# steidani/ConTrack

Hardware: AMD Instinct MI355X
Metric: timesteps/sec labeled+tracked (higher is better)
Workload: dtype f32 compare / int32 labels / int64 exact areas

## Files before the change

### contrack_amd/_native.py

```python
import ctypes as C
import os
import weakref

import numpy as np

from . import _abi

_HERE = os.path.dirname(os.path.abspath(__file__))
LIB_PATH = os.environ.get("CTK_LIB", os.path.join(_HERE, "libcontrack_hip.so"))
INCLUDE_DIR = os.environ.get("CTK_INCLUDE", os.path.join(os.path.dirname(_HERE), "include"))
_lib = None

CMP_OPS = {">=": 0, "ge": 0, "<=": 1, "le": 1, ">": 2, "gt": 2, "<": 3, "lt": 3}
GORL_ERRMSG = ' Please select from [>, >=, <, >=] for gorl'

TIMER_NAMES = ["k_threshold", "k_scan", "k_label2d", "k_overlap", "k_extent", "k_run_values", "k_relabel",
               "k_resolve", "k_resolve_final", "k_count", "host_seam_driver", "d2h", "h2d", "total"]


class ContrackHipError(RuntimeError):
    pass


def _headers():
# ... 150 lines not shown

def _subset_table(table):
    off, ids = table
    off, ids = np.ascontiguousarray(off, dtype=np.int64), np.ascontiguousarray(ids, dtype=np.int32)
    if off.ndim != 1 or ids.ndim != 1 or len(off) < 2:
        raise ValueError("a table is (off, ids): off int64 with 2 or T + 1 entries, ids int32")
    return off, ids


def _subset_kind(kind):
    if kind not in SUBSET_KINDS:
        raise ValueError("kind={!r}: 'id' or 'mask'".format(kind))
    return SUBSET_KINDS[kind]


class _SubsetCall:

    def __init__(self, table, invert, kind, want_hits=True):
        self.off, self.ids = _subset_table(table)
        self.hits = np.zeros(len(self.ids), dtype=np.uint64) if want_hits else None
        self.n = C.c_int64(0)
        self.table = (self.off.ctypes.data, len(self.off), self.ids.ctypes.data, len(self.ids), int(bool(invert)), _subset_kind(kind))

    def counts(self):
        return _ptr(self.hits), C.byref(self.n)


BLOCKSTAT_FORMS = ("row_lds", "row_glb")
BLOCK_WANTS = {"shape": ABI.constants["CTK_BLOCK_SHAPE"], "peaks": ABI.constants["CTK_BLOCK_PEAKS"]}
BLOCK_ROW = _dtype("ctk_block_row")


def _block_want(want):
    if isinstance(want, (int, np.integer)):
        return int(want)
    names = (want,) if isinstance(want, str) else tuple(want)
    unknown = [w for w in names if w not in BLOCK_WANTS]
    if unknown or not names:
        raise ValueError("want={!r}: 'shape', 'peaks' or both".format(want))
    return sum(BLOCK_WANTS[w] for w in set(names))


def blockstat_plan(want, longest, ny, nx, steps=1, elem_bytes=4, aligned=True, grid_max=0):
    v = np.zeros(14, dtype=np.int64)
    check(lib().ctk_debug_blockstat_plan(_block_want(want), int(elem_bytes), int(longest), int(ny), int(nx), int(steps), int(bool(aligned)), int(grid_max),
                                         v.ctypes.data))
    return dict(zip(("form", "vec", "vpt", "lds", "bps", "blocks", "grid", "xcd", "passes", "words", "entry", "lds_budget", "lds_entries", "part_lanes"),
                    (int(a) for a in v)))


class _BlockstatCall:

    def __init__(self, table, want):
        self.off, self.ids = _subset_table(table)
        self.rows = np.zeros(len(self.ids), dtype=BLOCK_ROW)
        self.args = (self.off.ctypes.data, len(self.off), self.ids.ctypes.data, len(self.ids), _block_want(want), self.rows.ctypes.data)


def lwa_plan(elem_bytes, rows, nx, ndom=1, steps=1, aligned=True):
    v = np.zeros(12, dtype=np.int64)
    check(lib().ctk_debug_lwa_plan(int(elem_bytes), int(rows), int(nx), int(ndom), int(steps), int(bool(aligned)), v.ctypes.data))
    return dict(zip(("ok", "vec", "strip", "nstrips", "lds", "lds_sel", "blocks", "grid", "xcd", "sel_blocks", "sel_grid", "sel_xcd"), (int(a) for a in v)))


def composite_plan(elem_bytes, npix, unroll=-1):
    v = np.zeros(3, dtype=np.int64)
    check(lib().ctk_debug_composite_plan(int(elem_bytes), int(npix), int(unroll), v.ctypes.data))
    return dict(unroll=int(v[0]), blocks=int(v[1]), grid=int(v[2]))


def centred_plan(elem_bytes, nbins, hy, hx, max_bin=0, kept=None, form=-1, unroll=-1, threads=-1):
    v = np.zeros(6, dtype=np.int64)
    check(lib().ctk_debug_centred_plan(int(elem_bytes), int(nbins), int(hy), int(hx), int(max_bin), int(max_bin if kept is None else kept), int(form),
                                       int(unroll), int(threads), v.ctypes.data))
    return dict(form=int(v[5]), unroll=int(v[0]), threads=int(v[1]), parts=int(v[2]), blocks=int(v[3]), grid=int(v[4]))


def forms(T, ny, nx, nt=None, aligned16=True, async_passes=24, n_cus=256, **query):
    q = FormQuery(T=T, nt=T if nt is None else nt, ny=ny, nx=nx, aligned16=int(aligned16), async_passes=async_passes, n_cus=n_cus,
                  **{k: int(v) for k, v in query.items()})
    p = FormPlan()
    check(lib().ctk_debug_forms(C.byref(q), C.byref(p)))
    return {n: getattr(p, n) for n, _ in FormPlan._fields_}


def debug_live():
    out = (C.c_int64 * 4)()
    check(lib().ctk_debug_live(out))
    return tuple(out)


def lib():
    global _lib
    if _lib is not None:
        return _lib
    if not os.path.exists(LIB_PATH):
        raise ContrackHipError(
            "libcontrack_hip.so not found at %s -- build it with `python -c 'import __graft_entry__ as g; g.build()'` "
            "or `make -C contrack_amd/csrc`; the HIP path has no CPU fallback" % LIB_PATH)
    L = C.CDLL(LIB_PATH)
    missing = [name for name in ABI.functions if not hasattr(L, name)]
    if missing:
        raise ContrackHipError("%s does not export %s, which the headers in %s declare" % (LIB_PATH, ", ".join(missing), INCLUDE_DIR))
    for name, (restype, argtypes) in ABI.functions.items():
        fn = getattr(L, name)
        fn.restype, fn.argtypes = restype, argtypes
    _lib = L
    return L


def _seg_starts(segments):
    st = np.asarray(segments)
    if st.ndim != 1 or (st.size and st.dtype.kind not in "iu"):
        raise ValueError("segment starts must be a 1-D integer array")
    return np.ascontiguousarray(st, dtype=np.int64)


def _thr_or_field(thr, T):
    if thr is None:
        return None
    thr = np.ascontiguousarray(thr, dtype=np.float64)
    if thr.shape != (T,):
        raise ValueError("thr must have shape (T,) and wrow (ny,)")
    return thr


def _groups(group, T, ngroups=None):
    if group is None:
        return None, 1 if ngroups is None else int(ngroups)
    g = np.asarray(group)
    if g.ndim != 1 or g.shape[0] != T:
        raise ValueError("group must hold one id per timestep (%d), not shape %s" % (T, g.shape))
    if g.dtype.kind not in "iu":
        raise ValueError("group ids must be integers")
    if g.size and (g.min() < np.iinfo(np.int32).min or g.max() > np.iinfo(np.int32).max):
        raise ValueError("group ids beyond int32")
    g = np.ascontiguousarray(g, dtype=np.int32)
    return g, (int(g.max()) + 1 if g.size else 1) if ngroups is None else int(ngroups)


def _level_weights(weights, nlev):
    w = np.ascontiguousarray(weights, dtype=np.float64)
    if w.ndim != 1 or w.shape[0] != nlev:
        raise ValueError("weights must hold one value per level (%d), not shape %s" % (nlev, w.shape))
    if not np.all(np.isfinite(w)) or np.any(w < 0):
        raise ValueError("each weight must be finite and >= 0")
    if not np.any(w > 0):
        raise ValueError("all weights are zero: no level is selected")
    return w


def _reversal_rows(rows, ny):
    second = rows.get("eq2") is not None
    if second != (rows.get("tS2") is not None):
        raise ValueError("eq2 and tS2 go together (both or neither)")
    keep = []
    for key, dt in (("eq", np.int32), ("po", np.int32), ("eq2", np.int32), ("dE", np.float64), ("tS", np.float64), ("tN", np.float64), ("tS2", np.float64)):
        if key in ("eq2", "tS2") and not second:
            keep.append(None)
            continue
        a = np.ascontiguousarray(rows[key], dtype=dt)
        if a.shape != (ny,):
            raise ValueError("rows[%r] must hold one value per latitude row (%d), not shape %s" % (key, ny, a.shape))
        keep.append(a)
    return [_ptr(a) for a in keep], keep

# ... 1599 lines not shown
            if not isinstance(field_source, np.memmap) or field_source.dtype not in (np.float32, np.float64):
                field_source = np.ascontiguousarray(field_source, dtype=np.float64 if np.asarray(field_source).dtype == np.float64 else np.float32)
            if field_source.ndim != 3:
                raise ValueError("field must be (time, lat, lon)")
        if shape is None:
            have = [a.shape for a in (flag_source, field_source) if not callable(a)]
            if not have:
                raise ValueError("reader callbacks need shape=(T, ny, nx) and dtype")
            shape = have[0]
        T, ny, nx = (int(v) for v in shape)
        for a in (flag_source, field_source):
            if not callable(a) and a.shape != (T, ny, nx):
                raise ValueError("flag and field must share one (time, lat, lon) shape")
        if callable(field_source):
            if dtype is None:
                raise ValueError("a field reader needs dtype")
            dt = np.dtype(dtype)
        else:
            dt = field_source.dtype
        if dt not in (np.dtype(np.float32), np.dtype(np.float64)):
            raise ValueError("the field must be float32 or float64")
        wrow = np.ascontiguousarray(wrow, dtype=np.float32)
        if wrow.shape != (ny,):
            raise ValueError("wrow must have shape (ny,)")
        tr = _Trampolines()

        def pk(_user, rows, n, idx, nidx):
            view = np.ctypeslib.as_array(C.cast(rows, C.POINTER(C.c_byte)), shape=(n * LIFE_ROW.itemsize,)).view(LIFE_ROW)
            chosen = np.ascontiguousarray(pick(view), dtype=np.int64).reshape(-1)
            if len(chosen) > n:
                raise ValueError("pick returned more indices than rows")
            np.ctypeslib.as_array(C.cast(idx, C.POINTER(C.c_int64)), shape=(max(int(n), 1),))[:len(chosen)] = chosen
            C.cast(nidx, C.POINTER(C.c_int64))[0] = len(chosen)
        pcb = tr.wrap(LIFE_PICK_FN, pk) if pick is not None else LIFE_PICK_FN()
        n, nx_ = C.c_int64(0), C.c_int64(0)
        tail = (wrow.ctypes.data, int(chunk_steps), pcb, None, C.byref(n), C.byref(nx_))
        if arrays:
            fn = L.ctk_lifecycle_stream_f64 if dt == np.float64 else L.ctk_lifecycle_stream_f32
            rc = fn(self._h, flag_source.ctypes.data, field_source.ctypes.data, T, ny, nx, *tail)
        else:
            fcb, vcb = tr.reader(flag_source, C.c_int32, (ny, nx)), tr.reader(field_source, _float_ctype(dt), (ny, nx))
            rc = L.ctk_lifecycle_stream_cb(self._h, dt.itemsize, T, ny, nx, fcb, None, vcb, None, *tail)
        tr.finish(rc)
        rows = self._life_rows(int(n.value))
        idx = np.empty(int(nx_.value), dtype=np.int64)
        exact = np.empty(int(nx_.value), dtype=LIFE_EXACT)
        check(L.ctk_lifecycle_stream_exact(self._h, idx.ctypes.data, exact.ctypes.data, len(idx)))
        return rows, idx, exact

    def debug_lifecycle_path(self, T):
        v = np.zeros(8, dtype=np.int64)
        steps = np.zeros(max(int(T), 1), dtype=np.uint8)
        check(lib().ctk_debug_lifecycle_path(self._h, v.ctypes.data, steps.ctypes.data, int(T)))
        return dict(zip("rw nsx nby vec given_up launches attempts sort".split(), (int(x) for x in v))), steps[:int(T)]

    def lifecycle_dev(self, flag_dev, field_dev, T, ny, nx, wrow, f64=False):
        wrow = np.ascontiguousarray(wrow, dtype=np.float32)
        n = C.c_int64(0)
        fn = lib().ctk_lifecycle_f64_dev if f64 else lib().ctk_lifecycle_f32_dev
        check(fn(self._h, flag_dev, field_dev, T, ny, nx, wrow.ctypes.data, C.byref(n)))
        return self._life_rows(int(n.value))

    def set_timing(self, level=2):
        check(lib().ctk_set_timing(self._h, 2 if level is True else int(level)))

    def set_fused(self, enable=True):
        check(lib().ctk_set_fused_pass(self._h, int(bool(enable))))

    def set_result_transfer(self, mode=-1):
        check(lib().ctk_set_result_transfer(self._h, int(mode)))
        self._transfer_mode = int(mode)

    @property
    def result_as_runs(self):
        m = getattr(self, "_transfer_mode", -1)
        if m >= 0:
            return m == 1
        import re
        v = os.environ.get("CTK_RLE_OUT")
        mt = re.match(r"\s*[+-]?\d+", v) if v is not None else None
        return v is None or (mt is not None and int(mt.group(0)) != 0)

    def stats(self):
        v = np.zeros(37, dtype=np.int64)
        check(lib().ctk_get_stats_n(self._h, v.ctypes.data, 37))
        names = ["runs", "max_runs_per_step", "components", "pairs", "seam_rows_to_driver", "labels_3d", "seam_ops",
                 "filter_passes", "host_path", "seam_loop_ns", "seam_folds", "seam_copy_ns", "ungrouped_pairs", "pair_table_regrows", "filter_rounds",
                 "ambiguous_decisions", "exact_fixups", "shared_seam_rows", "off_fused_path_reason", "relabel_kernel", "fused_pass", "x4_speculated", "result_as_runs", "mask_allocations_tried", "mask_ratio_x1000",
                 "mask_check_us", "mask_spacer_mb", "label_forms", "overlap_form", "rowcount_threads",
                 "filter_forms", "extent_form", "runval_form", "relabel_shape", "count_form", "device_cus", "rowcount_groups"]
        return dict(zip(names, v.tolist()))

    def debug_set_pair_capacity(self, records):
        check(lib().ctk_debug_set_pair_capacity(self._h, int(records)))

    def debug_set_seam_caps(self, labels, ops):
        check(lib().ctk_debug_set_seam_caps(self._h, int(labels), int(ops)))

    def debug_shard_exchange(self):
        v = np.zeros(12, dtype=np.int64)
        check(lib().ctk_debug_shard_exchange(self._h, v.ctypes.data))
        lo, hi = (lambda x: int(x) & 0xffffffff), (lambda x: (int(x) >> 32) & 0xffffffff)
        return dict(capB=int(v[0]), capB_repeats=int(v[1]), nlast=lo(v[2]), nh=hi(v[2]), capC=lo(v[3]), capD=hi(v[3]), x5_repeats=int(v[4]),
                    sent_records=lo(v[5]), sent_labels=hi(v[5]), ne=int(v[6]), pack_ext_workgroups=int(v[7]), tables_ahead_used=int(v[8]),
                    form=int(v[9]), shared_ops=int(v[10]), zero_exchanged=int(v[11]))

    def debug_set_shared_ops_reserve(self, n):
        check(lib().ctk_debug_set_shared_ops_reserve(self._h, int(n)))

    def debug_set_spin(self, limit_ms=0.0, stall_mode=0):
        check(lib().ctk_debug_set_spin(self._h, float(limit_ms), int(stall_mode)))

    def debug_set_mailbox(self, cand_records, labels):
        check(lib().ctk_debug_set_mailbox(self._h, int(cand_records), int(labels)))

    def set_filter_round(self, passes):
        check(lib().ctk_set_filter_round(self._h, int(passes)))

    def set_device_resolve(self, on=True):
        check(lib().ctk_set_device_resolve(self._h, int(bool(on))))

    def timing_sums(self, reset=True):
        sums = np.zeros(len(TIMER_NAMES), dtype=np.float64)
        cnt = np.zeros(len(TIMER_NAMES), dtype=np.int64)
        check(lib().ctk_get_timing_sums(self._h, sums.ctypes.data, cnt.ctypes.data, int(bool(reset))))
        return ({k: (float(v) / int(n) if n else 0.0) for k, v, n in zip(TIMER_NAMES, sums, cnt)}, dict(zip(TIMER_NAMES, cnt.tolist())))

    def time_relabel(self, flag_dev, persistence, variant, xcd=-1, reps=5):
        ms = np.zeros(reps, dtype=np.float64)
        check(lib().ctk_debug_time_relabel(self._h, flag_dev, int(persistence), int(variant), int(xcd), int(reps), ms.ctypes.data))
        return ms

    def stream_ceiling(self, ptr, nbytes, write, reps=5):
        ms = C.c_double(0.0)
        check(lib().ctk_debug_stream_ceiling(self._h, ptr, int(nbytes), int(write), int(reps), C.byref(ms)))
        return ms.value

    def timings(self):
        ms = np.zeros(len(TIMER_NAMES), dtype=np.float64)
        check(lib().ctk_get_timings(self._h, ms.ctypes.data))
        return dict(zip(TIMER_NAMES, ms.tolist()))

    def shard_label2d(self, anom_dev, T, ny, nx, thr, cmp_op, wrow, has_prev, f64=False):
        thr = None if thr is None else np.ascontiguousarray(thr, dtype=np.float64)
        wrow = np.ascontiguousarray(wrow, dtype=np.float32)
        fn = lib().ctk_shard_label2d_f64 if f64 else lib().ctk_shard_label2d
        check(fn(self._h, anom_dev, T, ny, nx, _ptr(thr), int(cmp_op), wrow.ctypes.data, int(bool(has_prev))))

    def halo_size(self):
        s = C.c_size_t(0)
        check(lib().ctk_shard_halo_size(self._h, C.byref(s)))
        return int(s.value)

    def halo_export(self):
        p, s = C.c_void_p(), C.c_size_t(0)
        check(lib().ctk_shard_halo_export(self._h, C.byref(p), C.byref(s)))
        return p, int(s.value)

    def halo_import(self, blob_dev, nbytes):
        check(lib().ctk_shard_halo_import(self._h, blob_dev, int(nbytes)))

    def shard_overlap(self):
        check(lib().ctk_shard_overlap(self._h))

    def shard_tables(self):
        p, s = C.c_void_p(), C.c_size_t(0)
        check(lib().ctk_shard_tables(self._h, C.byref(p), C.byref(s)))
        return C.string_at(p, s.value)

    def shard_extents(self, result, shard, t_begin):
        p, n = C.c_void_p(), C.c_int64(0)
        check(lib().ctk_shard_extents(self._h, result.ptr, int(shard), int(t_begin), C.byref(p), C.byref(n)))
        return p, int(n.value)

# ... 15 lines not shown
```

### contrack_amd/csrc/ctk_api.hip

```cpp
#include "ctk_kernels.hip"
#include "ctk_resolve_dev.hip"
#include "ctk_seam_dev.hip"
#include "ctk_lifecycle.hip"
#include "ctk_seam.h"
#include "ctk_comm.h"
#include "ctk_forms.h"
#include "ctk_select.h"
#include "ctk_own.h"
#include "../../include/contrack_hip_debug.h"

#include <chrono>
#include <cmath>
#include <cstdio>
#include <cstdlib>
#include <cstring>
#include <algorithm>
#include <vector>
#include <sys/mman.h>
#include <emmintrin.h>
#include <atomic>
#include <thread>
#include <functional>
#include <memory>
#include <mutex>
// ... 141 lines not shown
    ~RlePool() { crew.shutdown(); drop(); }
    void drop() { for (BounceLane &l : lane) l.release(); ready = false; }
    bool init(size_t need)
    {
        if (ready && need <= cap) return true;
        drop();
        cap = std::max(kRleBuf, (need + ((size_t)1 << 20) - 1) & ~(((size_t)1 << 20) - 1));
        for (BounceLane &l : lane)
            if (!l.create(cap)) { drop(); return false; }
        ready = true;
        return true;
    }
};

struct StreamIO {
    const void *host_in = nullptr;
    ctk_read_chunk_fn read = nullptr;
    void *read_user = nullptr;
    int32_t *host_out = nullptr;
    ctk_write_chunk_fn write = nullptr;
    void *write_user = nullptr;
    void *host_out_v = nullptr;
    ctk_write_values_fn write_v = nullptr;
    const void *host_in2 = nullptr;
    ctk_read_chunk_fn read2 = nullptr;
    void *read2_user = nullptr;
    size_t esz2 = 0;
    const void *dev2 = nullptr;
    bool ahead = false;
    int64_t chunk = 0;
    size_t esz = 4;
    double ms_read = 0, ms_write = 0, ms_in = 0, ms_out = 0;
    int64_t passes_in = 0;
};

struct LaunchKnobs {
    int form = -1;
    int64_t grid = 0;
    int xcd_dbg = -1;
    int64_t grid_dbg = 0;
    int64_t cap() const { return grid_dbg > 0 ? grid_dbg : CTK_LEVEL_GRID_MAX; }
    int xcd(int planned) const { return xcd_dbg >= 0 ? xcd_dbg : planned; }
    void launched(int f, int64_t g) { form = f; grid = g; }
};

struct ResidentSlab {
    DevBuf buf;
    int64_t T = -1; int ny = 0, nx = 0; bool f64 = false;
    uint64_t gen = 0;
    void drop() { T = -1; gen++; }
    void keep(int64_t T_, int ny_, int nx_, bool f64_) { T = T_; ny = ny_; nx = nx_; f64 = f64_; }
    bool held() const { return T >= 1 && buf.p; }
    void *find(int64_t T_, int ny_, int nx_, bool f64_) const
    {
        return held() && T == T_ && ny == ny_ && nx == nx_ && f64 == f64_ ? buf.p : nullptr;
    }
    void report(int64_t *T_, int *ny_, int *nx_, int *is_f64) const
    {
        if (T_) *T_ = T;
        if (ny_) *ny_ = ny;
        if (nx_) *nx_ = nx;
        if (is_f64) *is_f64 = f64 ? 1 : 0;
    }
    void adopt(DevBuf &other, int64_t T_, int ny_, int nx_, bool f64_) { buf.swap(other); gen++; keep(T_ >= 1 ? T_ : -1, ny_, nx_, f64_); }
    void release() { buf.release(); drop(); }
};

struct ctk_handle {
    int device = 0;
    int n_cus = 256;
    Stream stream;
    Stream side[2];
    Stream copy_stream;
    Event ev_fork, ev_join[2];
    Event ev_scan;
    State state = ST_IDLE;
    int64_t T = 0;
    int ny = 0, nx = 0, W = 0, has_prev = 0, cmp_op = 0;
    int32_t wshift = 0, limb_bits = CTK_LIMB_BITS_MIN;
    uint32_t total_runs = 0, max_runs_step = 0, total_comps = 0;
    uint32_t pair_cap = 0, seam_cap = 0;
    bool need_glb = false;
    DevBuf mask, wstart, rowstart, tcount, run_base, ncomp, cprefix, thr32, wlo, whi, counters;
    DevBuf run_comp, run_val, cs_mrep, cs_box, cs_area, d_mrep, d_box, d_area, comp_label;
    DevBuf g_x0, g_x1, g_y, g_parent, g_root, g_idmap, g_rs;
    DevBuf pairs, seams, ext, ops, op_first, op_next, op_stage, halo_in, halo_out, dbg;
    DevBuf seam_cnt, seam_off, d_seams, d_comp_t, pair_base, pair_cnt, rv_tdirty, d_blob, seam_rowoff;
    DevBuf rv_prc, rv_prd, rv_pgc, rv_pgd, rv_F, rv_B, rv_keep0, rv_keep1, rv_changed, rv_parent, rv_isroot, rv_rank, rv_lab, rv_lab_root, rv_lbox,
        rv_bsum, rv_boff, rv_cand_cnt, rv_cand_off, rv_cand, rv_cand_scratch, rv_seam_res, rv_scalars, rv_mark, rv_inv, rv_ff, rv_dmap, rv_dorig, rv_dbox, rv_inex, rv_touch;
    DevBuf lc_rows, lc_cnt, lc_wlo, lc_whi, lc_w, lc_work, lc_ovf, lc_ekeys, lc_offs, lc_sw, lc_sp, lc_out, lc_cross, lc_gtab, lc_occ, lc_cp;
    const int32_t *lc_flag = nullptr; const void *lc_field = nullptr;
    int lc_own = 0; uint64_t lc_io_gen = 0, lc_an_gen = 0;
    bool lc_f64 = false; int64_t lc_T = 0; int lc_ny = 0, lc_nx = 0;
    int64_t lc_path_T = -1; CtkLifePlan lc_plan = {0, 0, 0, 0, 0};
    int64_t lc_given_up = 0, lc_fb_launches = 0; int lc_attempts = 0, lc_sort = 0;
    std::vector<uint8_t> lc_rounds;
    bool lc_streamed = false;
    std::vector<int64_t> lx_idx;
    std::vector<ctk_life_exact> lx_rec;
    DevBuf chunk_vals;
    DevBuf sd_parent, sd_tmin, sd_tmax, sd_root, sd_nops, sd_lbox, rv_pstate, ci_bsum, scan_bsum;
    uint32_t *h_amail = nullptr;
    PinBuf amail_pin;
    uint32_t op_cap_hint = 4096;
    uint32_t nd_hint = 4096;
    int async_passes = 24;
    int use_async = -1;
    int async_off_ny = -1, async_off_nx = -1;
    uint32_t fz_pslot = 0;
    bool fz_init = false;
    bool in_one_call = false;
    bool guard_on = false;
    ResidentSlab an_slab;
    DevBuf an_clim, an_raw, an_idx;
    DevBuf an_acc, an_valid;
    int an_form = -1;
    int64_t an_waves_dbg = 0, an_gy_dbg = 0;
    int64_t an_last[6] = {0, 0, 0, 0, 0, 0};
    int64_t an_launches = 0;
    int64_t an_pct_n = -1;
    ResidentSlab lv_slab;
    DevBuf lv_tab;
    LaunchKnobs lv_knobs;
    DevBuf fl_tab, fl_out;
    int64_t fl_waves_dbg = 0, fl_gy_dbg = 0; int fl_form_dbg = -1;
    int64_t fl_last[8] = {-1, 0, 0, 0, 0, 0, 0, 0};
    int64_t fl_launches = 0;
    DevBuf gr_tab;
    LaunchKnobs gr_knobs;
    DevBuf lw_tab, lw_ref;
    LaunchKnobs lw_knobs;
    DevBuf sb_tab, sb_hits;
    LaunchKnobs sb_knobs;
    int sb_vec = 0;
    DevBuf bs_acc, bs_rows;
    LaunchKnobs bs_knobs;
    int bs_vec = 0;
    DevBuf io_in, io_out;
    uint64_t io_gen = 0;
    struct StreamIO *sio = nullptr;
    Event ev_h2d[2], ev_thr[2], ev_rel[2], ev_d2h[2];
    PinPair pin_in, pin_out;
    double stream_ms[4] = {0, 0, 0, 0};
    std::unique_ptr<BouncePool> bounce;
    std::unique_ptr<RlePool> rle;
    std::vector<uint32_t> rle_run_base;
    std::vector<RleBlock> rle_blocks;
    bool rle_out = false;
    int rle_mode = -1;
    DevBuf sh_mask_next, sh_send, sh_recv, sh_prev, sh_elist, sh_ovr_slot, sh_ovr_val, sh_amb_list, sh_counts, sh_cl_shared, sh_cl_sent;
    uint32_t sh_stamp_seq = 0;
    int sh_dev_off_ny = -1, sh_dev_off_nx = -1;
    std::unique_ptr<ShardScratch, ShardScratchFree> shard;
    uint32_t *h_mail2 = nullptr;
    PinBuf mail2_pin;
    PinBuf h_shard, h_lab, h_seam;
    bool halo_in_zero = false; void *halo_in_zero_p = nullptr; size_t halo_in_zero_cap = 0;
    uint32_t sh_capB = 0, sh_capC = 0, sh_capD = 0;
    int64_t sh_dbg[12] = {0};
    bool sh_dbg_valid = false;
    std::vector<std::pair<int32_t, int32_t>> sh_pairs;
    bool halo_valid = false, halo_v2 = false;
    std::vector<ctk_life_row> lc_host, lc_tmp;
    std::vector<std::pair<uint64_t, uint32_t>> lc_keys;
    std::vector<uint32_t> lc_cnt_host;
    PinBuf h_cand;
    PinBuf h_ops;
    PinBuf h_mail;
    uint32_t *h_mail1 = nullptr;
    PinBuf mail1_pin;
    PinBuf h_stage;
    uint32_t rb_last = 0, rb_total = 0;
    std::vector<double> c_thr; std::vector<float> c_w;
    int64_t c_T = -1; bool c_f64 = false, c_thr_valid = false, c_w_valid = false; int c_cmp = -1, c_w_nx = -1;
    DevBuf fld_raw, fld_f32, fld_pos, fld_order;
    int64_t fld_T = -1, fld_np = 0; int fld_ny = 0, fld_nx = 0, fld_esz = 0;
    int fld_prep_op = -1;
    int64_t fld_order_chunk = -1;
    std::vector<int32_t> fld_pos_host, fld_order_host;
    std::vector<int64_t> seg_starts;
    DevBuf seg_edge;
    std::vector<uint8_t> seg_edge_host;
    int64_t seg_edge_T = -1;
    const uint8_t *seg_cur = nullptr;
    const uint8_t *seg_cur_host = nullptr;
    std::vector<int64_t> seg_call;
    bool seg_shard_breaks = false;
    DevBuf fq_counts, fq_group;
    DevBuf sp_out, sp_words, sp_carry;
    std::vector<uint32_t> sp_words_host;
    int64_t sp_slice_dbg = 0;
    DevBuf cp_sum, cp_n;
    int cp_unroll_dbg = -1, cp_unroll = 0; int64_t cp_grid = 0;
    DevBuf ce_sum, ce_n, ce_idx;
    int ce_form_dbg = -1, ce_unroll_dbg = -1, ce_threads_dbg = -1, ce_form = 0, ce_unroll = 0, ce_threads = 0; int64_t ce_grid = 0;
    DevBuf bd_cols, bd_sec, bd_tab;
    int bd_form_dbg = -1, bd_rows_dbg = -1, bd_form = -1, bd_rows = 0; int64_t bd_grid = 0;
    PinPair bd_pin;
    DevBuf pc_hist, pc_buf;
    int64_t pc_sweeps = 0;
    int pc_groups = 0; size_t pc_slots = 0;
    DevBuf pf_out, pf_idx;
    int pf_form = -1; int64_t pf_max_pool = 0;
    DevBuf sf_out, sf_idx;
    int sf_tile = -1; int64_t sf_max_pool = 0;
    int64_t fq_slice_dbg = 0; int fq_nt = -1;
    int w_minlsb = 0;
    int64_t last_alive = 0, last_nlab = 0;
    int64_t rowoff_T = -1; int rowoff_ny = -1; void *rowoff_p = nullptr;
    uint32_t runs_cap = 0;
    CtkVariantSet spec_set = {false, false, false, false, false, false};
    int spec_ny = -1, spec_nx = -1; int64_t spec_T = -1;
    size_t mail_cap_c = 0, mail_cap_d = 0, mail_want_c = 0, mail_want_d = 0;
    const int32_t *d_op_next = nullptr;
    int use_device_resolve = 1;
    int filter_round = CTK_JACOBI_ROUND;
    uint32_t debug_pair_cap = 0;
    uint32_t debug_mail_c = 0, debug_mail_d = 0;
    int debug_sd_lab = 0, debug_sd_ops = 0;
    int debug_fail_stage = 0;
    int64_t debug_sh_gops = 0;
    uint64_t spin_limit = CTK_SPIN_LIMIT_TICKS;
    int debug_stall = 0;
    bool no_sys = false, sh_retrying = false;
    int small_threads[3] = {0, 0, 0};
    bool thr_nostore = false;
    bool thr_probe = false;
    bool rel_probe = false;
    int rel_variant = -1;
    bool mask_check_pending = false;
    int mask_check_retries = 0;
    int mask_tries = 0; double mask_ratio = 0.0;
    double mask_check_ms = 0; double mask_spacer_gb = 0;
    int xcd_rel_tuned = -1;
    int64_t rel_tuned_T = -1; int rel_tuned_ny = 0, rel_tuned_nx = 0; const void *rel_tuned_flag = nullptr;
    int64_t rel_seen_T = -1; int rel_seen_ny = 0, rel_seen_nx = 0;
    bool sh_collective_err = false;
    ctk_comm *active_comm = nullptr;
    SeamDriver sd, sd_glob;
    std::vector<int32_t> sd_last;
    std::vector<CtkOp> sd_ops;
    std::vector<unsigned char> sd_cand;
    int64_t stats[CTK_NSTATS_ALL] = {0};
    double ms_sum[CTK_NTIMERS] = {0};
    int64_t ms_cnt[CTK_NTIMERS] = {0};
    PinBuf h_blob;
    size_t h_blob_bytes = 0;
    PinBuf h_small;
    int64_t n_labels = 0, t_begin = 0;
    int32_t nops = 0;
    int timing = 0;
    uint64_t pass_no = 0;
    Event ev[CTK_K_COUNT + 2][2];
    bool ev_used[CTK_K_COUNT + 2];
    double ms[CTK_NTIMERS];
    bool ev_ready = false;
};

namespace {

int ensure(ctk_handle *h, DevBuf &b, size_t need)
{
    if (need == 0) need = 8;
    if (b.cap >= need) return CTK_OK;
    if (b.p && h && h->active_comm) { if (int rc = ctk_comm_wait(h->active_comm)) return rc; }
    b.release();
    hipError_t e = b.alloc(need + need / 8 + 256);
    if (e != hipSuccess) e = b.alloc(need);
    if (e != hipSuccess) return ctk_set_error(CTK_E_NOMEM, "hipMalloc(%zu bytes) failed: %s", need, hipGetErrorString(e));
    return CTK_OK;
}

int ensure_host(ctk_handle *h, PinBuf &b, size_t need, bool non_coherent = false)
{
    if (b.cap >= need && b.p) return CTK_OK;
    if (b.p && h && h->active_comm) { if (int rc = ctk_comm_wait(h->active_comm)) return rc; }
    b.release();
    const size_t c = need + need / 4 + 4096;
    const hipError_t e = b.alloc(c, non_coherent ? hipHostMallocNonCoherent : hipHostMallocDefault);
    if (e != hipSuccess) return ctk_set_error(CTK_E_NOMEM, "hipHostMalloc(%zu bytes) failed: %s", c, hipGetErrorString(e));
    return CTK_OK;
}

struct ActiveComm {
    ctk_handle *h;
    ActiveComm(ctk_handle *h_, ctk_comm *c) : h(h_) { h->active_comm = (c && c->world > 1) ? c : nullptr; }
    ~ActiveComm() { h->active_comm = nullptr; }
};

static int claim_io(ctk_handle *h, DevBuf &b, size_t need)
{
    h->io_gen++;
    return ensure(h, b, need);
}

template <typename T>
T *P(const DevBuf &b) { return (T *)b.p; }
inline uint32_t *CPX(const ctk_handle *h) { return (uint32_t *)h->cprefix.p + 1; }

struct Timer {
    ctk_handle *h;
    int k;
    bool on() const
    {
        return h->ev_ready && (h->timing >= 2 || (h->timing == 1 && ((k == CTK_K_THRESHOLD && (h->pass_no & 3) == 0) || (k == CTK_K_RELABEL && (h->pass_no & 3) == 2))));
    }
    Timer(ctk_handle *h_, int k_) : h(h_), k(k_)
// ... 86 lines not shown
{
    if (!h || enable < 0 || enable > 2) return ctk_set_error(CTK_E_INVALID, "ctk_set_timing: null handle or level not in 0..2");
    HIPCHK(hipSetDevice(h->device));
    if (enable && !h->ev_ready) {
        for (int k = 0; k <= CTK_KI_ROWCOUNT; k++) { HIPCHK(h->ev[k][0].create()); HIPCHK(h->ev[k][1].create()); }
        h->ev_ready = true;
    }
    h->timing = enable;
    return CTK_OK;
}

#ifdef CTK_PHASE_TIMING
extern "C" int ctk_debug_phase_times(unsigned long long *out)
{
    return hipMemcpyFromSymbol(out, HIP_SYMBOL(g_phase_t), sizeof(unsigned long long) * 16) == hipSuccess ? 0 : -1;
}
extern "C" int ctk_debug_rel_times(unsigned long long *out)
{
    if (hipDeviceSynchronize() != hipSuccess) return -1;
    return hipMemcpyFromSymbol(out, HIP_SYMBOL(g_rel_t), sizeof(unsigned long long) * 16) == hipSuccess ? 0 : -1;
}
extern "C" int ctk_debug_rel_acc(unsigned long long *out, int reset)
{
    if (hipDeviceSynchronize() != hipSuccess) return -1;
    if (out && hipMemcpyFromSymbol(out, HIP_SYMBOL(g_rel_acc), sizeof(unsigned long long) * 4096) != hipSuccess) return -1;
    if (reset) { std::vector<unsigned long long> z(4096, 0ull); if (hipMemcpyToSymbol(HIP_SYMBOL(g_rel_acc), z.data(), 4096 * 8) != hipSuccess) return -1; }
    return 0;
}
extern "C" int ctk_debug_pb_times(unsigned long long *out, int reset)
{
    if (hipDeviceSynchronize() != hipSuccess) return -1;
    if (out && hipMemcpyFromSymbol(out, HIP_SYMBOL(g_pb_t), sizeof(unsigned long long) * 4096) != hipSuccess) return -1;
    if (reset) {
        std::vector<unsigned long long> z(4096, 0ull);
        for (int i = 0; i < 1024; i++) z[4 * i] = ~0ull;
        if (hipMemcpyToSymbol(HIP_SYMBOL(g_pb_t), z.data(), sizeof(unsigned long long) * 4096) != hipSuccess) return -1;
    }
    return 0;
}
#endif

extern "C" int ctk_get_stats(ctk_handle *h, int64_t *out)
{
    if (!h || !out) return ctk_set_error(CTK_E_INVALID, "null argument");
    memcpy(out, h->stats, (size_t)CTK_NSTATS * sizeof(int64_t));
    return CTK_OK;
}
extern "C" int ctk_get_stats_n(ctk_handle *h, int64_t *out, int n)
{
    if (!h || !out || n < 0) return ctk_set_error(CTK_E_INVALID, "null argument");
    memcpy(out, h->stats, (size_t)std::min(n, CTK_NSTATS_ALL) * sizeof(int64_t));
    return CTK_OK;
}

extern "C" int ctk_debug_set_pair_capacity(ctk_handle *h, uint32_t records)
{
    if (!h) return ctk_set_error(CTK_E_INVALID, "null handle");
    h->debug_pair_cap = records;
    return CTK_OK;
}

extern "C" int ctk_debug_set_mailbox(ctk_handle *h, uint32_t cand_records, uint32_t labels)
{
    if (!h) return ctk_set_error(CTK_E_INVALID, "null handle");
    h->debug_mail_c = cand_records; h->debug_mail_d = labels;
    return CTK_OK;
}

extern "C" int ctk_debug_set_seam_caps(ctk_handle *h, int labels, int ops)
{
    if (!h || labels < 0 || ops < 0) return ctk_set_error(CTK_E_INVALID, "ctk_debug_set_seam_caps: null handle or negative capacity");
    h->debug_sd_lab = labels; h->debug_sd_ops = ops;
    h->async_off_ny = -1; h->async_off_nx = -1;
    h->sh_dev_off_ny = -1; h->sh_dev_off_nx = -1;
    return CTK_OK;
}

extern "C" int ctk_debug_set_small_threads(ctk_handle *h, int extent, int run_values, int compact_init)
{
    for (int v : {run_values, compact_init}) if (v != 0 && v != 64 && v != 128 && v != 256) return ctk_set_error(CTK_E_INVALID, "ctk_debug_set_small_threads: 0 / 64 / 128 / 256");
    if (extent != 0 && extent != 64 && extent != 128 && extent != 256 && extent != 1024) return ctk_set_error(CTK_E_INVALID, "ctk_debug_set_small_threads: extent 0 / 64 / 128 / 256, or 1024 = k_extent_blk");
    if (!h) return ctk_set_error(CTK_E_INVALID, "null handle");
    h->small_threads[0] = extent; h->small_threads[1] = run_values; h->small_threads[2] = compact_init;
    return CTK_OK;
}

static int launch_relabel(ctk_handle *h, int persistence, int32_t *flag_dev, bool with_fold, const int32_t *chunk_vals = nullptr, int64_t t0 = 0, int64_t nt = -1);
static int32_t *chunk_vals_for(ctk_handle *h, const int32_t *flag_dev, int *rows);
extern "C" int ctk_debug_time_relabel(ctk_handle *h, int32_t *flag_dev, int persistence, int variant, int xcd, int reps, double *ms)
{
    if (!h || !flag_dev || !ms || reps < 1 || variant < 0 || variant > 1) return ctk_set_error(CTK_E_INVALID, "ctk_debug_time_relabel: bad argument");
    if (h->state != ST_TABLES) return ctk_set_error(CTK_E_STATE, "ctk_debug_time_relabel needs a finished pass");
    HIPCHK(hipSetDevice(h->device));
    Event e0, e1;
    HIPCHK(e0.create());
    if (e1.create() != hipSuccess) return ctk_set_error(CTK_E_NODEVICE, "hipEventCreate failed");
    int rows = 0;
    const int32_t *cv = chunk_vals_for(h, flag_dev, &rows);
    const int keep_variant = h->rel_variant, keep_xcd = h->xcd_rel_tuned;
    h->rel_variant = variant;
    if (xcd >= 0) h->xcd_rel_tuned = xcd;
    int rc = CTK_OK;
    hipError_t err = hipSuccess;
    for (int r = 0; r < reps && rc == CTK_OK && err == hipSuccess; r++) {
        err = hipEventRecord(e0, h->stream);
        rc = launch_relabel(h, persistence, flag_dev, true, cv, 0, -1);
        if (err == hipSuccess) err = hipEventRecord(e1, h->stream);
        if (err == hipSuccess) err = hipEventSynchronize(e1);
        float f = 0.f;
        if (err == hipSuccess) err = hipEventElapsedTime(&f, e0, e1);
        ms[r] = f;
    }
    h->rel_variant = keep_variant; h->xcd_rel_tuned = keep_xcd;
    if (rc != CTK_OK) return rc;
    if (err != hipSuccess) return ctk_set_error(CTK_E_NODEVICE, "ctk_debug_time_relabel: %s", hipGetErrorString(err));
    return CTK_OK;
}

extern "C" int ctk_debug_forms(const ctk_form_query *q, ctk_form_plan *p)
{
    if (!q || !p) return ctk_set_error(CTK_E_INVALID, "ctk_debug_forms: null argument");
    if (q->T < 0 || q->nt < 0 || q->ny < 1 || q->nx < 1 || q->ny > 65535 || q->nx > 65535 || q->path < 0 || q->path > 2)
        return ctk_set_error(CTK_E_INVALID, "ctk_debug_forms: bad query (T=%lld nt=%lld ny=%lld nx=%lld path=%lld)", (long long)q->T, (long long)q->nt, (long long)q->ny,
                             (long long)q->nx, (long long)q->path);
    const int64_t T = q->T;
    const int ny = (int)q->ny, nx = (int)q->nx, W = (nx + 63) / 64;
    const CtkPath path = (CtkPath)q->path;
    auto set_of = [](int64_t b) { return CtkVariantSet{(b & 1) != 0, (b & 2) != 0, (b & 4) != 0, (b & 8) != 0, (b & 16) != 0, (b & 32) != 0}; };
    auto bits_of = [](const CtkVariantSet &v) { return (int64_t)((v.v1 ? 1 : 0) | (v.v2 ? 2 : 0) | (v.v3 ? 4 : 0) | (v.glb ? 8 : 0) | (v.one ? 16 : 0) | (v.v1hi ? 32 : 0)); };
    memset(p, 0, sizeof(*p));
    const CtkThrForm tf = ctk_threshold_form(q->nt, ny, nx, W, q->f64 != 0, q->aligned16 != 0, q->field != 0);
    p->thr_kind = tf.kind; p->thr_u7 = tf.u7; p->thr_rbt = tf.rbt; p->thr_grid = tf.grid;
    p->rowcount_threads = ctk_rowcount_threads(T, ny, W);
    const CtkLabelShape sh = ctk_label_shape(T, ny, W);
    p->v0b = sh.v0b; p->v0_ok = sh.v0_ok; p->v0_runs = sh.v0_runs;
    p->need_glb = ctk_label_need_glb((uint32_t)q->max_runs_step, ny);
    const CtkVariantSet sl = ctk_label_speculative(set_of(q->spec_set), sh);
    p->spec_launched = bits_of(sl); p->spec_bits = ctk_label_form_bits(sl, sh);
    const CtkLabelPlan lp = ctk_label_plan(T, ny, sh, (uint32_t)q->max_runs_step, set_of(q->launched));
    p->missing = bits_of(lp.missing); p->missing_bits = ctk_label_form_bits(lp.missing, sh); p->next_spec = bits_of(lp.next);
    p->overlap_form = ctk_overlap_form(T, ny, W) + (q->seg ? CTK_OVERLAP_SEG : 0);
    p->extent_form = ctk_extent_form(T, nx, (int)q->forced_extent);
    const CtkWritePlan wp = ctk_write_plan(T, q->nt, ny, nx, W, q->aligned16 != 0);
    p->write_kernel = wp.kernel; p->write_rb = wp.rb; p->write_sub = wp.sub; p->write_kb = wp.kb; p->write_batched = wp.tab_batched;
    p->write_lds = (int64_t)wp.lds; p->write_grid = wp.grid; p->write_shape = wp.shape;
    p->chunk_copy = ctk_write_chunk_copy(ctk_write_plan(T, T, ny, nx, W, q->aligned16 != 0));
    p->runval_threads = ctk_runval_threads(path, T, (uint64_t)q->total_runs, (int)q->forced_run_values);
    p->compact_init_threads = ctk_compact_init_threads(path, T, (int)q->forced_compact_init);
    p->count_staged = ctk_count_form_staged(q->n_labels);
    const CtkFilterPlan fp = ctk_filter_plan_fused(T, (int)q->async_passes, q->no_sys != 0, (int)q->n_cus, q->seg != 0, (int)q->pslot,
                                                   ctk_rank_blocks((size_t)q->total_runs));
    p->count_fused = ctk_count_form_fused(q->last_nlab, fp.passes);
    p->filter_sys = fp.sys; p->filter_passes = fp.passes; p->filter_blk = fp.round.blk; p->filter_two_pc = fp.round.two_pc; p->filter_nb = fp.round.nb;
    p->filter_unite = fp.unite; p->filter_merged = fp.merged; p->filter_bits = fp.bits; p->filter_bits_sync = ctk_filter_bits_sync(T, q->seg != 0);
    const CtkFilterRound fr = ctk_filter_round(T, (int)q->async_passes, q->no_sys != 0, (int)q->n_cus);
    p->round_blk = fr.blk; p->round_two_pc = fr.two_pc; p->round_nb = fr.nb;
    p->rowcount_groups = ctk_rowcount_groups((int)p->rowcount_threads, ny, W);
    return CTK_OK;
}

extern "C" int ctk_debug_live(int64_t *out4)
{
    if (!out4) return ctk_set_error(CTK_E_INVALID, "ctk_debug_live: null argument");
    for (int i = 0; i < CTK_LIVE_KINDS; i++) out4[i] = g_ctk_live[i].load();
    return CTK_OK;
}
// ... 265 lines not shown
    }
    e[(size_t)T_total - 1] |= 2u;
    bool any = false;
    for (int64_t t = t_begin; t < t_begin + T && !any; t++)
        any = (e[(size_t)t] & ~((t == 0 ? 1u : 0u) | (t == T_total - 1 ? 2u : 0u))) != 0;
    if (!any) return CTK_OK;
    CTKCHK(ensure(h, h->seg_edge, (size_t)T));
    HIPCHK(hipMemcpy(h->seg_edge.p, e.data() + t_begin, (size_t)T, hipMemcpyHostToDevice));
    h->seg_cur = P<uint8_t>(h->seg_edge);
    h->seg_cur_host = e.data() + t_begin;
    return CTK_OK;
}

static int prepare_field(ctk_handle *h, bool f64, int cmp_op, int64_t chunk)
{
    hipStream_t s = h->stream;
    const int64_t n = h->fld_np * h->fld_ny * h->fld_nx;
    if (!f64 && h->fld_esz == 8 && h->fld_prep_op != cmp_op) {
        CTKCHK(ensure(h, h->fld_f32, (size_t)n * 4));
        const int g = (int)std::min<int64_t>((n + 255) / 256, 8192);
        const double *in = P<double>(h->fld_raw);
        float *out = P<float>(h->fld_f32);
        switch (cmp_op) {
        case 0: k_thr_field_prep<0><<<g, 256, 0, s>>>(in, out, n); break;
        case 1: k_thr_field_prep<1><<<g, 256, 0, s>>>(in, out, n); break;
        case 2: k_thr_field_prep<2><<<g, 256, 0, s>>>(in, out, n); break;
        default: k_thr_field_prep<3><<<g, 256, 0, s>>>(in, out, n); break;
        }
        HIPCHK(hipGetLastError());
        h->fld_prep_op = cmp_op;
    }
    if (h->fld_order_chunk != chunk) {
        const int64_t T = h->fld_T;
        std::vector<int32_t> &ord = h->fld_order_host;
        ord.resize((size_t)std::max<int64_t>(T, 1));
        for (int64_t c0 = 0; c0 < T; c0 += chunk) {
            const int64_t nt = std::min<int64_t>(chunk, T - c0);
            int32_t *o = ord.data() + c0;
            for (int64_t i = 0; i < nt; i++) o[i] = (int32_t)i;
            const int32_t *p = h->fld_pos_host.data() + c0;
            std::stable_sort(o, o + nt, [p](int32_t a, int32_t b) { return p[a] < p[b]; });
        }
        CTKCHK(ensure(h, h->fld_order, ord.size() * 4));
        HIPCHK(hipMemcpyAsync(h->fld_order.p, ord.data(), ord.size() * 4, hipMemcpyHostToDevice, s));
        h->fld_order_chunk = chunk;
    }
    return CTK_OK;
}

struct Label2dCall {
    const void *anom_dev; bool f64; int64_t T; int ny, nx, W; const double *thr; int cmp_op; const float *wrow;
    bool defer_compact;
    bool fld_call;
    int64_t nrows;
    bool same_thr, same_w;
    double *thr32; int64_t *wlo;
    size_t w_bytes;
    bool mask_fresh;
    uint32_t scan_stamp;
    CtkLabelShape shape;
    bool spec;
    CtkVariantSet launched;
    int rc_launched, rc_groups; int64_t label_forms;
};

static int label2d_begin(ctk_handle *h, Label2dCall &c, int has_prev)
{
    const int64_t T = c.T;
    const int ny = c.ny, nx = c.nx;
    c.fld_call = T > 0 && !c.thr && h->fld_T == T && h->fld_ny == ny && h->fld_nx == nx;
    if (T > 0 && !c.thr && !c.fld_call && ny >= 1 && nx >= 1)
        return ctk_set_error(CTK_E_INVALID, "ctk_shard_label2d: thr is NULL and no threshold field of shape (T=%lld, ny=%d, nx=%d) is set%s", (long long)T, ny, nx,
                             h->fld_T >= 0 ? " (the field set has another shape)" : "");
    if (T < 0 || ny < 1 || nx < 1 || (T > 0 && ((!c.anom_dev && !h->sio) || (!c.thr && !c.fld_call))) || !c.wrow)
        return ctk_set_error(CTK_E_INVALID, "ctk_shard_label2d: bad shape (T=%lld ny=%d nx=%d) or null pointer", (long long)T, ny, nx);
    if (c.cmp_op < 0 || c.cmp_op > 3) return ctk_set_error(CTK_E_INVALID, "ctk_shard_label2d: cmp_op %d not in 0..3", c.cmp_op);
    if (nx > 65535 || ny > 65535) return ctk_set_error(CTK_E_RANGE, "ctk_shard_label2d: grid %dx%d exceeds 65535 per axis", ny, nx);
    if (T > 4000000ll) return ctk_set_error(CTK_E_RANGE, "ctk_shard_label2d: more than 4 000 000 timesteps in one shard");
    HIPCHK(hipSetDevice(h->device));
    memset(h->ms, 0, sizeof(h->ms));
    h->pass_no++;
    h->state = ST_IDLE;
    h->halo_valid = false; h->halo_v2 = c.defer_compact;
    h->T = T; h->ny = ny; h->nx = nx; h->W = (nx + 63) / 64; h->has_prev = has_prev ? 1 : 0; h->cmp_op = c.cmp_op;
    c.W = h->W;
    c.nrows = T * ny;
    c.shape = ctk_label_shape(T, ny, c.W);
    c.spec = false;
    c.launched = {false, false, false, false, false, false};
    c.rc_launched = 0; c.rc_groups = 0; c.label_forms = 0;
    return CTK_OK;
}

static int label2d_stage_inputs(ctk_handle *h, Label2dCall &c)
{
    const int64_t T = c.T;
    const int ny = c.ny, nx = c.nx, cmp_op = c.cmp_op;
    const bool f64 = c.f64;
    const double *thr = c.thr;
    const float *wrow = c.wrow;
    const size_t thr_bytes = (size_t)std::max<int64_t>(T, 1) * 8;
    c.same_thr = c.fld_call || (h->c_thr_valid && h->c_T == T && h->c_f64 == f64 && h->c_cmp == cmp_op && (T == 0 || memcmp(h->c_thr.data(), thr, (size_t)T * 8) == 0));
    if (c.fld_call) h->c_thr_valid = false;
    c.same_w = h->c_w_valid && (int)h->c_w.size() == ny && h->c_w_nx == nx && memcmp(h->c_w.data(), wrow, (size_t)ny * 4) == 0;
    double *thr32 = nullptr;
    int64_t *wlo = nullptr;
    c.w_bytes = (size_t)ny * 16 + ((size_t)ny + 2) * 4;
    if (!c.same_thr || !c.same_w) {
        CTKCHK(ensure_host(h, h->h_stage, thr_bytes + c.w_bytes));
        thr32 = (double *)h->h_stage.p;
        wlo = (int64_t *)((char *)h->h_stage.p + thr_bytes);
    }
    c.thr32 = thr32; c.wlo = wlo;
    if (!c.same_thr) {
        h->c_thr_valid = false;
        if (f64) for (int64_t t = 0; t < T; t++) thr32[t] = thr[t];
        else for (int64_t t = 0; t < T; t++) ((float *)thr32)[t] = adjust_threshold(thr[t], cmp_op);
        h->c_thr.assign(thr, thr + T);
        h->c_T = T; h->c_f64 = f64; h->c_cmp = cmp_op;
    }
    if (!c.same_w) {
        h->c_w_valid = false;
        CTKCHK(ctk_weights_to_limbs(wrow, ny, (int64_t)ny * nx, wlo, wlo + ny, &h->wshift, &h->limb_bits));
        h->c_w.assign(wrow, wrow + ny);
        h->c_w_nx = nx;
        std::vector<int> lsb((size_t)ny, 127);
        int maxbl = 0;
        h->w_minlsb = 127;
        for (int y = 0; y < ny; y++) {
            const __int128 wi = (__int128)wlo[y] + ((__int128)wlo[ny + y] << h->limb_bits);
            if (wi == 0) continue;
            unsigned __int128 m = wi < 0 ? (unsigned __int128)(-wi) : (unsigned __int128)wi;
            int l = 0, bl = 0;
            while (!((m >> l) & 1)) l++;
            for (unsigned __int128 q = m; q; q >>= 1) bl++;
            lsb[(size_t)y] = l;
            maxbl = std::max(maxbl, bl);
            h->w_minlsb = std::min(h->w_minlsb, l);
        }
        if (h->w_minlsb == 127) h->w_minlsb = 0;
        int lg = 0;
        while (((int64_t)1 << lg) < (int64_t)ny * nx) lg++;
        int32_t *next_tiny = (int32_t *)(wlo + 2 * (size_t)ny);
        next_tiny[ny] = ny;
        for (int y = ny - 1; y >= 0; y--) next_tiny[y] = (lsb[(size_t)y] < maxbl + lg - 53) ? y : next_tiny[y + 1];
    }
    return CTK_OK;
}

static int label2d_upload(ctk_handle *h, Label2dCall &c)
{
    const int64_t T = c.T, nrows = c.nrows;
    const int W = c.W;
    hipStream_t s = h->stream;
    const void *mask_before = h->mask.p;
    CTKCHK(ensure(h, h->mask, (size_t)nrows * W * 8));
    c.mask_fresh = h->mask.p != mask_before;
    CTKCHK(ensure(h, h->wstart, (size_t)nrows * W * 2));
    CTKCHK(ensure(h, h->rowstart, (size_t)nrows * 4));
    CTKCHK(ensure(h, h->tcount, (size_t)T * 4));
    CTKCHK(ensure(h, h->run_base, (size_t)(T + 1) * 4));
    CTKCHK(ensure(h, h->ncomp, (size_t)T * 4));
    CTKCHK(ensure(h, h->cprefix, (size_t)(T + 2) * 4));
    CTKCHK(ensure(h, h->thr32, (size_t)T * 8));
    CTKCHK(ensure(h, h->wlo, c.w_bytes));
    CTKCHK(ensure(h, h->counters, CTK_CNT_WORDS * 4));
    CTKCHK(ensure_host(h, h->h_small, (size_t)(T + 1) * 4 + 1024));
// ... 90 lines not shown
            HIPCHK(hipEventSynchronize(e1));
            float f = 0.f;
            HIPCHK(hipEventElapsedTime(&f, e0, e1));
            *ms = f;
            return CTK_OK;
        };
        int rc = CTK_OK;
        double ro_ms = 0.0, best_ms = 1e30;
        const double accept = 1.085;
        h->thr_probe = true;
        struct ProbeOff { ctk_handle *h; ~ProbeOff() { h->thr_probe = false; h->thr_nostore = false; } } probe_off{h};
        h->thr_nostore = true;
        rc = time_it(&ro_ms);
        h->thr_nostore = false;
        if (rc == CTK_OK) rc = time_it(&best_ms);
        h->mask_tries = 1;
        if (rc == CTK_OK && best_ms > accept * ro_ms) {
            double ro2 = 0.0;
            h->thr_nostore = true;
            rc = time_it(&ro2);
            h->thr_nostore = false;
            if (rc == CTK_OK && (ro2 > 1.04 * ro_ms || ro_ms > 1.04 * ro2 || best_ms < 0.98 * std::min(ro_ms, ro2))) { best_ms = 0.0; h->mask_tries = 0; if (++h->mask_check_retries <= 3) h->mask_check_pending = true; }
            else ro_ms = std::min(ro_ms, ro2);
        } else if (rc == CTK_OK && best_ms < 0.98 * ro_ms) h->mask_tries = 0;
        const int max_tries = ctk_env().mask_tries;
        std::vector<DevBuf> held;
        for (int k = 0; rc == CTK_OK && k < max_tries && best_ms > accept * ro_ms; k++) {
            size_t mem_free = 0, mem_total = 0;
            const size_t spacer = (size_t)1 << 30;
            if (hipMemGetInfo(&mem_free, &mem_total) != hipSuccess || mem_free < spacer + mbytes + mem_total / 4) { (void)hipGetLastError(); break; }
            DevBuf sp;
            if (sp.alloc(spacer) != hipSuccess) { (void)hipGetLastError(); break; }
            held.push_back(std::move(sp)); h->mask_spacer_gb = 1.0;
            DevBuf nb;
            if (ensure(h, nb, mbytes) != CTK_OK) break;
            h->mask.swap(nb);
            double ms = 0.0;
            rc = time_it(&ms);
            h->mask_tries++;
            if (rc == CTK_OK && ms < best_ms) best_ms = ms;
            else h->mask.swap(nb);
            held.push_back(std::move(nb));
        }
        h->mask_ratio = ro_ms > 0 ? best_ms / ro_ms : 0.0;
        if (ctk_env().hosttrace) fprintf(stderr, "mask placement: %d allocation(s) tried, threshold kernel on a %lld-step window %.4f ms = %.3f x its time without stores (%.4f), mask at %p, slab at %p\n", h->mask_tries, (long long)nt_probe, best_ms, h->mask_ratio, ro_ms, h->mask.p, anom_dev);
        for (DevBuf &b : held) b.release();
        if (rc != CTK_OK) return rc;
    }
    return CTK_OK;
}

static int label2d_threshold(ctk_handle *h, const Label2dCall &c)
{
    if (c.T == 0) return CTK_OK;
    Timer tm(h, CTK_K_THRESHOLD);
    CTKCHK(mask_placement_check(h, c));
    if (c.anom_dev) return launch_threshold(h, c, c.anom_dev, 0, c.T);
    return stream_in(h, c.f64, c.T, c.ny, c.nx, [&](const void *src, int64_t t0, int64_t nt) { return launch_threshold(h, c, src, t0, nt); });
}

struct RowcountInstance { void (*fn)(const uint64_t *, int, int, uint16_t *, uint32_t *, uint32_t *); int rcu; };
template <int RCU> static RowcountInstance rowcount_instance() { return {k_rowcount<RCU>, RCU}; }
static int label2d_rowcount(ctk_handle *h, Label2dCall &c)
{
    const int64_t T = c.T;
    c.scan_stamp = (uint32_t)(h->pass_no & 0x7fffffffu) | 0x80000000u;
    Timer tm(h, CTK_KI_ROWCOUNT);
    const int rc_threads = ctk_rowcount_threads(T, c.ny, c.W);
    const int rc_groups = ctk_rowcount_groups(rc_threads, c.ny, c.W);
    RowcountInstance ki = rowcount_instance<8>();
    switch (rc_groups) {
    case 4: ki = rowcount_instance<4>(); break;
    case 6: ki = rowcount_instance<6>(); break;
    default: break;
    }
    if (T > 0) ki.fn<<<(int)T, rc_threads, 0, h->stream>>>(P<uint64_t>(h->mask), c.ny, c.W, P<uint16_t>(h->wstart), P<uint32_t>(h->rowstart), P<uint32_t>(h->tcount));
    c.rc_launched = T > 0 ? rc_threads : 0;
    c.rc_groups = (T > 0 && ctk_rowcount_first_form(c.ny, c.W)) ? ki.rcu : 0;
    CTKCHK(launch_scan_u32(h, P<uint32_t>(h->tcount), T, P<uint32_t>(h->run_base), h->h_mail1, c.scan_stamp));
    HIPCHK(hipGetLastError());
    return CTK_OK;
}

static int launch_label2d(ctk_handle *h, Label2dCall &c, const CtkVariantSet &vs, uint32_t cap_runs)
{
    const int T = (int)c.T;
    hipStream_t s = h->stream;
    Label2dArgs a;
    a.mask = P<uint64_t>(h->mask); a.wstart = P<uint16_t>(h->wstart); a.rowstart = P<uint32_t>(h->rowstart);
    a.run_base = P<uint32_t>(h->run_base); a.run_comp = P<uint32_t>(h->run_comp); a.ncomp = P<uint32_t>(h->ncomp);
    a.cs_mrep = P<uint32_t>(h->cs_mrep); a.cs_box = P<uint32_t>(h->cs_box); a.cs_area = P<int64_t>(h->cs_area);
    a.seams = P<CtkSeam>(h->seams); a.seam_cnt = P<uint32_t>(h->seam_cnt); a.counters = P<uint32_t>(h->counters);
    a.wlo = P<int64_t>(h->wlo); a.whi = P<int64_t>(h->wlo) + h->ny;
    a.ny = c.ny; a.nx = c.nx; a.W = c.W; a.lds_cap = CTK_LDS_RUNS; a.cap_runs = cap_runs;
    a.g_x0 = P<uint16_t>(h->g_x0); a.g_x1 = P<uint16_t>(h->g_x1); a.g_y = P<uint16_t>(h->g_y);
    a.g_parent = P<uint32_t>(h->g_parent); a.g_root = P<uint32_t>(h->g_root); a.g_idmap = P<uint32_t>(h->g_idmap);
    if (vs.one) k_label2d_lds<CTK_LDS_RUNS, 512, -1, 1024><<<T, 1024, 0, s>>>(a);
    if (vs.v2 || vs.v3) HIPCHK(hipEventRecord(h->ev_fork, s));
    if (vs.v1) {
        if (c.shape.v0b) k_label2d_lds<CTK_LBL_V0B_RUNS, 272, -1, 256, 256><<<T, 256, 0, s>>>(a);
        else if (c.shape.v0_ok) k_label2d_lds<CTK_LBL_V0_RUNS, 240, -1, 256, 256><<<T, 256, 0, s>>>(a);
        else k_label2d_lds<CTK_LBL_V1_RUNS, 288, -1, 256><<<T, 256, 0, s>>>(a);
    }
    if (vs.v1hi) {
        if (c.shape.v0b) k_label2d_lds<CTK_LBL_V1_RUNS, 288, CTK_LBL_V0B_RUNS, 256><<<T, 256, 0, s>>>(a);
        else k_label2d_lds<CTK_LBL_V1_RUNS, 288, CTK_LBL_V0_RUNS, 256><<<T, 256, 0, s>>>(a);
    }
    c.label_forms |= ctk_label_form_bits(vs, c.shape);
    if (vs.v2) {
        HIPCHK(hipStreamWaitEvent(h->side[0], h->ev_fork, 0));
        k_label2d_lds<CTK_LBL_V2_RUNS, 512, CTK_LBL_V1_RUNS, 512><<<T, 512, 0, h->side[0]>>>(a);
        HIPCHK(hipEventRecord(h->ev_join[0], h->side[0]));
    }
    if (vs.v3) {
        HIPCHK(hipStreamWaitEvent(h->side[1], h->ev_fork, 0));
        k_label2d_lds<CTK_LDS_RUNS, 512, CTK_LBL_V2_RUNS, 1024><<<T, 1024, 0, h->side[1]>>>(a);
        HIPCHK(hipEventRecord(h->ev_join[1], h->side[1]));
    }
    if (vs.v2) HIPCHK(hipStreamWaitEvent(s, h->ev_join[0], 0));
    if (vs.v3) HIPCHK(hipStreamWaitEvent(s, h->ev_join[1], 0));
    if (vs.glb) k_label2d_glb<<<T, 256, 0, s>>>(a, P<uint32_t>(h->g_rs));
    HIPCHK(hipGetLastError());
    return CTK_OK;
}

static int label2d_speculate(ctk_handle *h, Label2dCall &c)
{
    const int64_t T = c.T, nrows = c.nrows;
    if (nrows > 0x7fffffff) return ctk_set_error(CTK_E_RANGE, "ctk_shard_label2d: more than 2^31 rows in one shard");
    h->seam_cap = (uint32_t)nrows;
    CTKCHK(ensure(h, h->seams, (size_t)nrows * sizeof(CtkSeam)));
    CTKCHK(ensure(h, h->seam_cnt, (size_t)T * 4));
    CTKCHK(ensure(h, h->seam_off, (size_t)(T + 1) * 4));
    c.spec = T > 0 && h->runs_cap > 0 && h->spec_ny == c.ny && h->spec_nx == c.nx && (!h->spec_set.glb || h->spec_T >= T);
    if (c.spec) {
        Timer tm(h, CTK_K_LABEL2D);
        c.launched = ctk_label_speculative(h->spec_set, c.shape);
        CTKCHK(launch_label2d(h, c, c.launched, h->runs_cap));
    }
    return CTK_OK;
}

static int label2d_wait_scan(ctk_handle *h, const Label2dCall &c)
{
    HT("thr+scan launched");
    {
        volatile uint32_t *vm = h->h_mail1;
        for (uint64_t spins = 0; vm[4] != c.scan_stamp; spins++) {
            if ((spins & 0xfffff) == 0xfffff) {
                const hipError_t q = hipStreamQuery(h->stream);
                if (q == hipSuccess) { if (vm[4] != c.scan_stamp) return ctk_set_error(CTK_E_INTERNAL, "stage 1: the run scan did not report"); break; }
                if (q != hipErrorNotReady) return ctk_set_error(CTK_E_NODEVICE, "stage 1: %s", hipGetErrorString(q));
            }
        }
        __atomic_thread_fence(__ATOMIC_ACQUIRE);
    }
    const uint32_t m_total = h->h_mail1[0], m_max = h->h_mail1[1], m_ovf = h->h_mail1[2], m_last = h->h_mail1[3];
    HT("sync1 done");
    if (m_ovf & CTK_OVF_RUNS) return ctk_set_error(CTK_E_RANGE, "ctk_shard_label2d: more than 2^32-1 runs in one shard");
    h->total_runs = m_total;
    h->max_runs_step = m_max;
    h->rb_total = m_total; h->rb_last = m_total - m_last;
    h->need_glb = ctk_label_need_glb(h->max_runs_step, c.ny);
    memset(h->stats, 0, sizeof(h->stats));
    h->stats[CTK_S_RUNS] = h->total_runs; h->stats[CTK_S_MAX_RUNS_STEP] = h->max_runs_step;
    h->stats[CTK_S_MASK_TRIES] = h->mask_tries; h->stats[CTK_S_MASK_RATIO] = (int64_t)(h->mask_ratio * 1000.0 + 0.5);
    h->stats[CTK_S_MASK_CHECK_US] = (int64_t)(h->mask_check_ms * 1000.0 + 0.5); h->stats[CTK_S_MASK_SPACER_MB] = (int64_t)(h->mask_spacer_gb * 1024.0 + 0.5);
    return CTK_OK;
}

static int label2d_regrow(ctk_handle *h, Label2dCall &c)
{
    const size_t R = h->total_runs;
    const bool fits = c.spec && R <= h->runs_cap;
    if (!fits) {
        const size_t Rc = R + R / 8 + 1024;
        CTKCHK(ensure(h, h->run_comp, Rc * 4));
        CTKCHK(ensure(h, h->run_val, Rc * 4));
        CTKCHK(ensure(h, h->cs_mrep, Rc * 4));
        CTKCHK(ensure(h, h->cs_box, Rc * 16));
        CTKCHK(ensure(h, h->cs_area, Rc * 16));
        CTKCHK(ensure(h, h->d_mrep, Rc * 4));
        CTKCHK(ensure(h, h->d_box, Rc * 8));
        CTKCHK(ensure(h, h->d_area, Rc * 16));
        CTKCHK(ensure(h, h->d_comp_t, Rc * 4));
        if (h->need_glb || h->spec_set.glb) {
            CTKCHK(ensure(h, h->g_x0, Rc * 2)); CTKCHK(ensure(h, h->g_x1, Rc * 2)); CTKCHK(ensure(h, h->g_y, Rc * 2));
            CTKCHK(ensure(h, h->g_parent, Rc * 4)); CTKCHK(ensure(h, h->g_root, Rc * 4)); CTKCHK(ensure(h, h->g_idmap, Rc * 4));
        }
        h->runs_cap = (uint32_t)std::min<size_t>(Rc, 0xffffffffu);
        c.launched = {false, false, false, false, false, false};
        if (c.spec) c.label_forms |= CTK_LABEL_DISCARDED;
    }
    if (c.defer_compact) {
        const size_t Rd = (size_t)h->runs_cap + (size_t)c.ny * ((size_t)c.nx / 2 + 1);
        CTKCHK(ensure(h, h->d_mrep, Rd * 4)); CTKCHK(ensure(h, h->d_box, Rd * 8)); CTKCHK(ensure(h, h->d_area, Rd * 16)); CTKCHK(ensure(h, h->d_comp_t, Rd * 4));
    }
    if (h->need_glb) {
        const size_t Rc = h->runs_cap;
        CTKCHK(ensure(h, h->g_x0, Rc * 2)); CTKCHK(ensure(h, h->g_x1, Rc * 2)); CTKCHK(ensure(h, h->g_y, Rc * 2));
        CTKCHK(ensure(h, h->g_parent, Rc * 4)); CTKCHK(ensure(h, h->g_root, Rc * 4)); CTKCHK(ensure(h, h->g_idmap, Rc * 4));
        CTKCHK(ensure(h, h->g_rs, (size_t)c.T * (c.ny + 1) * 4));
    }
    return CTK_OK;
}

static int label2d_finish_labels(ctk_handle *h, Label2dCall &c)
{
    if (c.T > 0) {
        const CtkLabelPlan p = ctk_label_plan(c.T, c.ny, c.shape, h->max_runs_step, c.launched);
        if (ctk_variants_any(p.missing)) {
            HT("before label2d launch");
            Timer tm(h, CTK_K_LABEL2D);
            CTKCHK(launch_label2d(h, c, p.missing, h->runs_cap));
        }
        h->spec_set = p.next;
        h->spec_ny = c.ny; h->spec_nx = c.nx; h->spec_T = c.T;
    }
    h->stats[CTK_S_LABEL_FORMS] = c.label_forms; h->stats[CTK_S_ROWCOUNT_THREADS] = c.rc_launched; h->stats[CTK_S_ROWCOUNT_GROUPS] = c.rc_groups; h->stats[CTK_S_DEVICE_CUS] = h->n_cus;
    return CTK_OK;
}

static int label2d_compact(ctk_handle *h, const Label2dCall &c)
{
    const int64_t T = c.T;
    hipStream_t s = h->stream;
    h->fz_init = false;
    if (c.defer_compact) return CTK_OK;
    if (T > 0 && h->use_device_resolve && async_wanted(h)) {
        const size_t R = h->total_runs ? h->total_runs : 1;
        CTKCHK(ensure(h, h->rv_F, R * 16)); CTKCHK(ensure(h, h->rv_B, R * 16));
        CTKCHK(ensure(h, h->rv_keep0, R)); CTKCHK(ensure(h, h->rv_keep1, R));
        CTKCHK(ensure(h, h->rv_touch, R * 4)); CTKCHK(ensure(h, h->rv_parent, R * 4));
        CTKCHK(ensure(h, h->rv_changed, (size_t)(CTK_MAX_JACOBI + 8) * CTK_CHG_SLOTS * 4));
        CTKCHK(ensure(h, h->rv_scalars, 64));
        CTKCHK(ensure(h, h->rv_pstate, (size_t)(T + 1) * 4 * CTK_PSTATE_STRIDE));
        CompInit ci;
        ci.F = P<int64_t>(h->rv_F); ci.B = P<int64_t>(h->rv_B); ci.keep0 = P<uint8_t>(h->rv_keep0); ci.keep1 = P<uint8_t>(h->rv_keep1);
        ci.touch = P<uint32_t>(h->rv_touch); ci.parent = P<uint32_t>(h->rv_parent); ci.changed = P<uint32_t>(h->rv_changed);
        ci.ambig = P<uint32_t>(h->rv_scalars) + 1; ci.pstate = P<uint32_t>(h->rv_pstate);
        ci.next_tiny = (const int32_t *)(P<int64_t>(h->wlo) + 2 * (size_t)h->ny);
        ci.nchanged = (CTK_MAX_JACOBI + 1) * CTK_CHG_SLOTS; ci.pstride = CTK_PSTATE_STRIDE; ci.T = T;
        ci.base_ptr = nullptr; ci.ovr_slot = nullptr; ci.amb_cnt = nullptr; ci.dcount = nullptr; ci.bsum = nullptr;
        Timer tm(h, CTK_K_SCAN);
        if (T > 4 * CTK_CI_BLOCK) {
            const int nb = (int)((T + CTK_CI_BLOCK - 1) / CTK_CI_BLOCK);
            CTKCHK(ensure(h, h->ci_bsum, (size_t)nb * 4));
            k_sum_blocks<<<nb, CTK_CI_BLOCK, 0, s>>>(P<uint32_t>(h->ncomp), T, P<uint32_t>(h->ci_bsum));
            ci.bsum = P<uint32_t>(h->ci_bsum);
        }
        k_compact_init<<<(int)T, ctk_compact_init_threads(CTK_PATH_FUSED, T, h->small_threads[2]), 0, s>>>(
            P<uint32_t>(h->run_base), P<uint32_t>(h->ncomp), CPX(h), P<uint32_t>(h->cs_mrep), P<uint32_t>(h->cs_box), P<int64_t>(h->cs_area),
            P<uint32_t>(h->d_mrep), P<uint16_t>(h->d_box), P<int64_t>(h->d_area), P<uint32_t>(h->d_comp_t), ci);
        HIPCHK(hipGetLastError());
        h->fz_init = true;
    } else {
        Timer tm(h, CTK_K_SCAN);
        CTKCHK(launch_scan_u32(h, P<uint32_t>(h->ncomp), T, CPX(h)));
        HIPCHK(hipGetLastError());
        if (T > 0) {
            k_compact_comps<<<(int)T, 256, 0, s>>>(P<uint32_t>(h->run_base), P<uint32_t>(h->ncomp), CPX(h), P<uint32_t>(h->cs_mrep),
                                                   P<uint32_t>(h->cs_box), P<int64_t>(h->cs_area), P<uint32_t>(h->d_mrep), P<uint16_t>(h->d_box),
                                                   P<int64_t>(h->d_area), P<uint32_t>(h->d_comp_t));
            HIPCHK(hipGetLastError());
        }
    }
    return CTK_OK;
}

static int shard_label2d_impl(ctk_handle *h, const void *anom_dev, bool f64, int64_t T, int ny, int nx, const double *thr,
                              int cmp_op, const float *wrow, int has_prev, bool defer_compact = false)
{
    if (!h) return ctk_set_error(CTK_E_INVALID, "null handle");
    Label2dCall c = {};
    c.anom_dev = anom_dev; c.f64 = f64; c.T = T; c.ny = ny; c.nx = nx; c.thr = thr; c.cmp_op = cmp_op; c.wrow = wrow; c.defer_compact = defer_compact;
// ... 32 lines not shown
static size_t halo_max_bytes(const ctk_handle *h) { return halo_off_runcomp(h) + (size_t)h->ny * ((size_t)h->nx / 2 + 1) * 4; }

extern "C" int ctk_shard_halo_size(ctk_handle *h, size_t *max_bytes)
{
    if (!h || !max_bytes) return ctk_set_error(CTK_E_INVALID, "null argument");
    if (h->state < ST_LABELLED) return ctk_set_error(CTK_E_STATE, "ctk_shard_halo_size before ctk_shard_label2d");
    *max_bytes = halo_max_bytes(h);
    return CTK_OK;
}

extern "C" int ctk_shard_halo_export(ctk_handle *h, void **blob_dev, size_t *nbytes)
{
    if (!h || !blob_dev || !nbytes) return ctk_set_error(CTK_E_INVALID, "null argument");
    if (h->state < ST_LABELLED) return ctk_set_error(CTK_E_STATE, "ctk_shard_halo_export before ctk_shard_label2d");
    HIPCHK(hipSetDevice(h->device));
    CTKCHK(ensure(h, h->halo_out, halo_max_bytes(h)));
    char *dst = (char *)h->halo_out.p;
    hipStream_t s = h->stream;
    if (h->T > 0) {
        const int64_t t = h->T - 1;
        const uint32_t hb_t = h->rb_last, n = h->rb_total - h->rb_last;
        HIPCHK(hipMemcpyAsync(dst, P<uint64_t>(h->mask) + t * h->ny * h->W, (size_t)h->ny * h->W * 8, hipMemcpyDeviceToDevice, s));
        HIPCHK(hipMemcpyAsync(dst + halo_off_wstart(h), P<uint16_t>(h->wstart) + t * h->ny * h->W, (size_t)h->ny * h->W * 2, hipMemcpyDeviceToDevice, s));
        HIPCHK(hipMemcpyAsync(dst + halo_off_rowstart(h), P<uint32_t>(h->rowstart) + t * h->ny, (size_t)h->ny * 4, hipMemcpyDeviceToDevice, s));
        if (n) HIPCHK(hipMemcpyAsync(dst + halo_off_runcomp(h), P<uint32_t>(h->run_comp) + hb_t, (size_t)n * 4, hipMemcpyDeviceToDevice, s));
        *nbytes = halo_off_runcomp(h) + (size_t)n * 4;
    } else {
        HIPCHK(hipMemsetAsync(dst, 0, halo_off_runcomp(h), s));
        *nbytes = halo_off_runcomp(h);
    }
    HIPCHK(hipStreamSynchronize(s));
    *blob_dev = dst;
    return CTK_OK;
}

extern "C" int ctk_shard_halo_import(ctk_handle *h, const void *blob_dev, size_t nbytes)
{
    if (!h || !blob_dev) return ctk_set_error(CTK_E_INVALID, "null argument");
    if (h->state != ST_LABELLED) return ctk_set_error(CTK_E_STATE, "ctk_shard_halo_import needs a labelled shard");
    if (nbytes < halo_off_runcomp(h) || nbytes > halo_max_bytes(h)) return ctk_set_error(CTK_E_INVALID, "halo blob has %zu bytes, expected %zu..%zu", nbytes, halo_off_runcomp(h), halo_max_bytes(h));
    HIPCHK(hipSetDevice(h->device));
    CTKCHK(ensure(h, h->halo_in, halo_max_bytes(h)));
    h->halo_in_zero = false;
    HIPCHK(hipMemcpyAsync(h->halo_in.p, blob_dev, nbytes, hipMemcpyDeviceToDevice, h->stream));
    HIPCHK(hipStreamSynchronize(h->stream));
    h->halo_valid = true;
    return CTK_OK;
}

static int launch_overlap(ctk_handle *h)
{
    OverlapArgs a;
    a.mask = P<uint64_t>(h->mask); a.wstart = P<uint16_t>(h->wstart); a.rowstart = P<uint32_t>(h->rowstart); a.run_base = P<uint32_t>(h->run_base);
    a.run_comp = P<uint32_t>(h->run_comp);
    const char *hl = (const char *)h->halo_in.p;
    const size_t o0 = h->halo_v2 ? 16 : 0;
    a.halo_mask = (const uint64_t *)(hl ? hl + o0 : nullptr);
    a.halo_wstart = hl ? (const uint16_t *)(hl + o0 + halo_off_wstart(h)) : nullptr;
    a.halo_rowstart = hl ? (const uint32_t *)(hl + o0 + halo_off_rowstart(h)) : nullptr;
    a.halo_run_comp = hl ? (const uint32_t *)(hl + o0 + halo_off_runcomp(h)) : nullptr;
    a.has_prev = (h->has_prev && hl) ? 1 : 0;
    a.pairs = P<CtkPair>(h->pairs); a.pair_cap = h->pair_cap; a.counters = P<uint32_t>(h->counters);
    a.pair_base = P<uint32_t>(h->pair_base); a.pair_cnt = P<uint32_t>(h->pair_cnt);
    a.wlo = P<int64_t>(h->wlo); a.whi = P<int64_t>(h->wlo) + h->ny;
    a.ny = h->ny; a.nx = h->nx; a.W = h->W;
    a.cprefix = nullptr; a.mrep = nullptr; a.p_rc = nullptr; a.p_rd = nullptr; a.p_gc = nullptr; a.p_gd = nullptr; a.F = nullptr;
    a.pslot = 0; a.upair_cap = h->pair_cap;
    h->fz_pslot = 0;
    if (h->fz_init && (uint64_t)h->T * CTK_PSLOT + 4096 <= (uint64_t)h->pair_cap) {
        a.pslot = CTK_PSLOT; a.upair_cap = h->pair_cap - (uint32_t)(h->T * CTK_PSLOT);
        h->fz_pslot = CTK_PSLOT;
    }
    if (h->fz_init) {
        const size_t PC = h->pair_cap ? h->pair_cap : 1;
        CTKCHK(ensure(h, h->rv_prc, PC * 4)); CTKCHK(ensure(h, h->rv_prd, PC * 4)); CTKCHK(ensure(h, h->rv_pgc, PC * 4)); CTKCHK(ensure(h, h->rv_pgd, PC * 4));
        a.cprefix = CPX(h); a.mrep = P<uint32_t>(h->d_mrep); a.F = P<int64_t>(h->rv_F);
        a.p_rc = P<uint32_t>(h->rv_prc); a.p_rd = P<uint32_t>(h->rv_prd); a.p_gc = P<uint32_t>(h->rv_pgc); a.p_gd = P<uint32_t>(h->rv_pgd);
    }
    Timer tm(h, CTK_K_OVERLAP);
    OverlapArgsSeg as;
    static_cast<OverlapArgs &>(as) = a;
    as.seg_edge = h->seg_cur;
    const int form = ctk_overlap_form(h->T, h->ny, h->W);
#define CTK_OVERLAP(OVB, TH, WPE)                                                                        \
    case CTK_OVERLAP_CODE(OVB, TH, WPE):                                                                 \
        if (as.seg_edge) k_overlap<OVB, TH, WPE, true><<<(int)h->T, TH, 0, h->stream>>>(as);             \
        else k_overlap<OVB, TH, WPE><<<(int)h->T, TH, 0, h->stream>>>(a);                                \
        break
    switch (form) {
    CTK_OVERLAP(4, 128, 5);
    CTK_OVERLAP(4, 512, 1);
    CTK_OVERLAP(4, 256, 1);
    CTK_OVERLAP(5, 256, 1);
    CTK_OVERLAP(6, 256, 1);
    CTK_OVERLAP(8, 256, 1);
    default: return ctk_set_error(CTK_E_INTERNAL, "k_overlap: no instance of form %d", form);
    }
#undef CTK_OVERLAP
    h->stats[CTK_S_OVERLAP_FORM] = (as.seg_edge ? CTK_OVERLAP_SEG : 0) + form;
    HIPCHK(hipGetLastError());
    return CTK_OK;
}

extern "C" int ctk_shard_overlap(ctk_handle *h)
{
    if (!h) return ctk_set_error(CTK_E_INVALID, "null handle");
    if (h->state != ST_LABELLED) return ctk_set_error(CTK_E_STATE, "ctk_shard_overlap needs ctk_shard_label2d first");
    HIPCHK(hipSetDevice(h->device));
    if (h->has_prev && (!h->halo_in.p || !h->halo_valid))
        return ctk_set_error(CTK_E_STATE, "ctk_shard_overlap: has_prev set but no halo imported since ctk_shard_label2d");
    size_t want = (size_t)h->total_runs / 2 + (size_t)h->T * 8 + 4096;
    if (h->fz_init) want = std::max<size_t>(want, (size_t)h->T * CTK_PSLOT + (size_t)h->T * 8 + 8192);
    if (want > 0x7fffffffull) want = 0x7fffffffull;
    if (h->pair_cap < want || !h->pairs.p) {
        CTKCHK(ensure(h, h->pairs, want * sizeof(CtkPair)));
        h->pair_cap = (uint32_t)std::min<size_t>(h->pairs.cap / sizeof(CtkPair), 0x7fffffffull);
    }
    if (h->debug_pair_cap) { h->pair_cap = std::min(h->pair_cap, h->debug_pair_cap); h->debug_pair_cap = 0; }
    CTKCHK(ensure(h, h->pair_base, (size_t)h->T * 4));
    CTKCHK(ensure(h, h->pair_cnt, (size_t)h->T * 4));
    if (h->T > 0) CTKCHK(launch_overlap(h));
    h->state = ST_OVERLAPPED;
    return CTK_OK;
}

static int build_tables_blob(ctk_handle *h, bool to_device, const void **blob, size_t *nbytes)
{
    if (!h || !blob || !nbytes) return ctk_set_error(CTK_E_INVALID, "null argument");
    if (h->state != ST_OVERLAPPED && h->state != ST_TABLES) return ctk_set_error(CTK_E_STATE, "ctk_shard_tables needs ctk_shard_overlap first");
    HIPCHK(hipSetDevice(h->device));
    hipStream_t s = h->stream;
    const double t0 = now_ms();
    uint32_t *hc = (uint32_t *)h->h_small.p + (h->T + 2);
    uint32_t cnt[CTK_CNT_N], ctot = 0, stot = 0;
    CTKCHK(launch_scan_u32(h, P<uint32_t>(h->seam_cnt), h->T, P<uint32_t>(h->seam_off)));
    HIPCHK(hipGetLastError());
    for (int attempt = 0;; attempt++) {
        HIPCHK(hipMemcpyAsync(hc, h->counters.p, CTK_CNT_N * 4, hipMemcpyDeviceToHost, s));
        HIPCHK(hipMemcpyAsync(hc + CTK_CNT_N, CPX(h) + h->T, 4, hipMemcpyDeviceToHost, s));
        HIPCHK(hipMemcpyAsync(hc + CTK_CNT_N + 1, P<uint32_t>(h->seam_off) + h->T, 4, hipMemcpyDeviceToHost, s));
        HIPCHK(hipStreamSynchronize(s));
        memcpy(cnt, hc, sizeof(cnt));
        ctot = hc[CTK_CNT_N];
        stot = hc[CTK_CNT_N + 1];
        if (!(cnt[CTK_CNT_OVERFLOW] & CTK_OVF_PAIRS) && (uint64_t)cnt[CTK_CNT_PAIRS] + cnt[CTK_CNT_UPAIRS] <= h->pair_cap) break;
        if (attempt >= 6) return ctk_set_error(CTK_E_RANGE, "pair table keeps overflowing");
        h->stats[CTK_S_PAIR_REGROW]++;
        size_t want = std::max<size_t>((size_t)cnt[CTK_CNT_PAIRS] + cnt[CTK_CNT_UPAIRS] + 1024, (size_t)h->pair_cap * 2);
        if (want > 0xfffffff0ull) return ctk_set_error(CTK_E_RANGE, "pair table beyond 2^32 records");
        CTKCHK(ensure(h, h->pairs, want * sizeof(CtkPair)));
        h->pair_cap = (uint32_t)std::min<size_t>(h->pairs.cap / sizeof(CtkPair), 0xfffffff0ull);
        uint32_t zero[2] = {0, 0};
        HIPCHK(hipMemcpyAsync(P<uint32_t>(h->counters) + CTK_CNT_PAIRS, zero, 4, hipMemcpyHostToDevice, s));
        HIPCHK(hipMemcpyAsync(P<uint32_t>(h->counters) + CTK_CNT_UPAIRS, zero, 4, hipMemcpyHostToDevice, s));
        uint32_t ovf = cnt[CTK_CNT_OVERFLOW] & ~CTK_OVF_PAIRS;
        HIPCHK(hipMemcpyAsync(P<uint32_t>(h->counters) + CTK_CNT_OVERFLOW, &ovf, 4, hipMemcpyHostToDevice, s));
        HIPCHK(hipStreamSynchronize(s));
        h->fz_init = false;
        CTKCHK(launch_overlap(h));
    }
    h->total_comps = ctot;
    const int64_t T = h->T, NC = ctot, NPG = cnt[CTK_CNT_PAIRS], NPU = cnt[CTK_CNT_UPAIRS], NP = NPG + NPU, NS = stot;
    if (NS) {
        CTKCHK(ensure(h, h->d_seams, (size_t)NS * sizeof(CtkSeam)));
        k_compact_seams<<<(int)T, 256, 0, s>>>(P<CtkSeam>(h->seams), P<uint32_t>(h->seam_cnt), P<uint32_t>(h->seam_off), h->ny, P<CtkSeam>(h->d_seams));
        HIPCHK(hipGetLastError());
    }
    const size_t bytes = ctk_blob_bytes(T, NC, NP, NS);
    char *p;
    if (to_device) { CTKCHK(ensure(h, h->d_blob, bytes)); p = (char *)h->d_blob.p; }
    else { CTKCHK(ensure_host(h, h->h_blob, bytes)); p = (char *)h->h_blob.p; }
    const hipMemcpyKind kind = to_device ? hipMemcpyDeviceToDevice : hipMemcpyDeviceToHost;
    CtkBlobHeader hdr;
    memset(&hdr, 0, sizeof(hdr));
    hdr.magic = CTK_BLOB_MAGIC; hdr.T = T; hdr.ny = h->ny; hdr.nx = h->nx; hdr.wshift = h->wshift; hdr.limb_bits = h->limb_bits; hdr.has_prev = (h->has_prev && h->halo_in.p) ? 1 : 0;
    hdr.ncomps = NC; hdr.npairs = NP; hdr.nseams = NS; hdr.npairs_grouped = NPG;
    if (to_device) HIPCHK(hipMemcpyAsync(p, &hdr, sizeof(hdr), hipMemcpyHostToDevice, s)); else memcpy(p, &hdr, sizeof(hdr));
    p += sizeof(CtkBlobHeader);
    if (T) HIPCHK(hipMemcpyAsync(p, h->ncomp.p, (size_t)T * 4, kind, s));
    p += ctk_align8((size_t)T * 4);
    if (NC) HIPCHK(hipMemcpyAsync(p, h->d_mrep.p, (size_t)NC * 4, kind, s));
    p += ctk_align8((size_t)NC * 4);
// ... 2264 lines not shown
```

### contrack_amd/csrc/ctk_device.h

```cpp
#pragma once
#include <stdint.h>

#define CTK_CNT_PAIRS      0
#define CTK_CNT_SEAMS      1
#define CTK_CNT_OVERFLOW   2
#define CTK_CNT_WROTE_ZERO 3
#define CTK_CNT_ALIVE      4
#define CTK_CNT_UPAIRS     5
#define CTK_CNT_TICKET     6
#define CTK_CNT_POISON     8
#define CTK_CNT_NOPS       9
#define CTK_CNT_N          16
#define CTK_CNT_SUM_NC     16
#define CTK_CNT_SUM_NOPS   17
#define CTK_CNT_SUM_NP     18
#define CTK_CNT_ZEROED     24
#define CTK_ZF_OFF    64
#define CTK_ZF_SLOTS  1024
#define CTK_ZF_STRIDE 16
#define CTK_CNT_WORDS (CTK_ZF_OFF + CTK_ZF_SLOTS * CTK_ZF_STRIDE)

#define CTK_RB 16
#define RC_ROWS 2048
#define CTK_LDS_RUNS 4096
#define CTK_LDS_NY 1024
#define CTK_CV 64
#define CTK_CV_MAXCHUNK 1024
#define EX_TW 16
#define CTK_MAX_JACOBI 240
#define CTK_JACOBI_ROUND 10
#define PB_G 16
#define CTK_RL_BLOCKS 8192

#define CTK_OVF_PAIRS 1u
#define CTK_OVF_SEAMS 2u
#define CTK_OVF_RUNS  4u
```

### contrack_amd/csrc/ctk_forms.h

```cpp
#pragma once
#include <stdint.h>
#include <stddef.h>
#include <algorithm>
#include "ctk_device.h"

enum CtkPath { CTK_PATH_STAGED = 0, CTK_PATH_FUSED = 1, CTK_PATH_SHARDED = 2 };

inline int ctk_grid_for_rows(int64_t nrows) { return (int)std::min<int64_t>(std::max<int64_t>((nrows + 3) / 4, 1), 256 * 16); }

enum CtkThrKind {
    CTK_THR_V7 = 0,
    CTK_THR_V6,
    CTK_THR_F32,
    CTK_THR_F64,
    CTK_THR_FIELD_VEC,
    CTK_THR_FIELD_GEN
};
#define CTK_THR_XCD_TILE 64
struct CtkThrForm {
    int kind;
    int u7;
    int rbt;
    int r6, nchunk_t;
    int64_t nchunks;
// ... 19 lines not shown
        f.kind = CTK_THR_V7;
        f.grid = (unsigned)nblk4;
        const int L = (f.rbt * W * 16 + 255) / 256;
        int best = 1 << 30;
        for (int u = 8; u >= 4; u--) { const int waste = (L + u - 1) / u * u - L; if (waste < best) { best = waste; f.u7 = u; } }
    }
    return f;
}

inline int ctk_rowcount_threads(int64_t T, int ny, int W)
{
    return (W <= 64 && ny <= RC_ROWS && ny > 256 && T <= 2048) ? 512 : ((T > 65536 && (int64_t)ny * W <= 2048) ? 128 : 256);
}
inline int ctk_rowcount_groups(int threads, int ny, int W)
{
    if (W > 64) return 8;
    const int per_group = (threads / 64) * (64 / W), need = (ny + per_group - 1) / per_group;
    return need <= 4 ? 4 : need <= 6 ? 6 : 8;
}
inline bool ctk_rowcount_first_form(int ny, int W) { return W <= 64 && ny <= RC_ROWS; }

#define CTK_LBL_V0B_RUNS 768
#define CTK_LBL_V0_RUNS 832
#define CTK_LBL_V1_RUNS 1024
#define CTK_LBL_V2_RUNS 2048
struct CtkVariantSet { bool v1, v2, v3, glb, one, v1hi; };
inline bool ctk_variants_any(const CtkVariantSet &v) { return v.v1 || v.v2 || v.v3 || v.glb || v.one || v.v1hi; }
struct CtkLabelShape {
    bool v0b, v0_ok;
    uint32_t v0_runs;
};
inline CtkLabelShape ctk_label_shape(int64_t T, int ny, int W)
{
    CtkLabelShape s;
    s.v0b = ny <= 256 && (int64_t)ny * W > 960 && (int64_t)ny * W <= 1088;
    s.v0_ok = (T > 65536 && ny <= 256 && (int64_t)ny * W <= 960) || s.v0b;
    s.v0_runs = s.v0b ? CTK_LBL_V0B_RUNS : CTK_LBL_V0_RUNS;
    return s;
}
inline bool ctk_label_need_glb(uint32_t max_runs_step, int ny) { return max_runs_step > CTK_LDS_RUNS || ny > CTK_LDS_NY; }
inline CtkVariantSet ctk_label_speculative(const CtkVariantSet &spec_set, const CtkLabelShape &sh)
{
    CtkVariantSet v = spec_set;
    v.v1hi = spec_set.v1hi && sh.v0_ok;
    return v;
}
#define CTK_LABEL_DISCARDED 512
inline int64_t ctk_label_form_bits(const CtkVariantSet &vs, const CtkLabelShape &sh)
{
    return (vs.one ? 1 : 0) | (vs.v1 ? (sh.v0b ? 2 : sh.v0_ok ? 4 : 8) : 0) | (vs.v1hi ? (sh.v0b ? 16 : 32) : 0) | (vs.v2 ? 64 : 0) |
           (vs.v3 ? 128 : 0) | (vs.glb ? 256 : 0);
}
struct CtkLabelPlan {
    CtkVariantSet missing;
    CtkVariantSet next;
};
inline CtkLabelPlan ctk_label_plan(int64_t T, int ny, const CtkLabelShape &sh, uint32_t max_runs_step, const CtkVariantSet &launched)
{
    const bool glb = ctk_label_need_glb(max_runs_step, ny);
    const bool v2 = max_runs_step > CTK_LBL_V1_RUNS, v3 = max_runs_step > CTK_LBL_V2_RUNS;
    const bool prefer_one = T <= 512 && max_runs_step > CTK_LBL_V1_RUNS;
    const bool none_lds = !launched.v1 && !launched.v2 && !launched.v3 && !launched.one;
    CtkVariantSet need = {true, v2, v3, glb, false, sh.v0_ok && max_runs_step > sh.v0_runs};
    if ((prefer_one && none_lds) || launched.one) need = {false, false, false, glb, true, false};
    CtkLabelPlan p;
    p.missing = {need.v1 && !launched.v1, need.v2 && !launched.v2, need.v3 && !launched.v3, need.glb && !launched.glb, need.one && !launched.one,
                 need.v1hi && !launched.v1hi};
    if (prefer_one) p.next = {false, false, false, need.glb, true, need.v1hi};
    else p.next = {true, v2, v3, need.glb, false, need.v1hi};
    return p;
}

#define CTK_OVERLAP_CODE(OVB, TH, WPE) ((OVB) * 10000 + (TH) * 10 + (WPE))
#define CTK_OVERLAP_SEG 1000000
inline int ctk_overlap_form(int64_t T, int ny, int W)
{
    const int nwords = ny * W, per = (nwords + 255) / 256;
    if (T > 65536 && nwords <= 2048) return CTK_OVERLAP_CODE(4, 128, 5);
    if (T <= 1024 && nwords >= 8192) return CTK_OVERLAP_CODE(4, 512, 1);
    if (per <= 4 || per > 8) return CTK_OVERLAP_CODE(4, 256, 1);
    if (per == 5) return CTK_OVERLAP_CODE(5, 256, 1);
    if (per == 6) return CTK_OVERLAP_CODE(6, 256, 1);
    return CTK_OVERLAP_CODE(8, 256, 1);
}

#define CTK_EXTENT_BLK 1024
inline int ctk_extent_form(int64_t T, int nx, int forced)
{
    if (forced > 0) return forced;
    if (T > 2048) return nx < 1024 ? CTK_EXTENT_BLK : 128;
    return 256;
}

#define CTK_RV5 512
#define CTK_RVCAP 2048
enum CtkWriteKernel { CTK_WR_NONE = -1, CTK_WR_GENERIC = 0, CTK_WR_V4 = 4, CTK_WR_V5 = 5 };
inline int ctk_write_rows(int64_t T, int ny, int nx)
{
    const int n4r = std::max(1, nx / 4);
    int rb = std::min(ny, std::max(1, std::min(64, 1024 / n4r)));
    const int store_cap = n4r >= 256 ? 2304 : 6912;
    const int rb_max = std::min(ny, std::max(rb, std::min(96, store_cap / n4r)));
    while (rb < rb_max && T * ((ny + rb - 1) / rb) > 130000) rb++;
    while (rb < ny && T * ((ny + rb - 1) / rb) >= (1 << 24)) rb++;
    return rb;
}
inline size_t ctk_write_tables_lds(int rb, int W)
{
    return (size_t)rb * W * 8 + (((size_t)rb * W * 2 + 7) & ~(size_t)7) + ((((size_t)rb + 1) * 4 + 7) & ~(size_t)7);
}
struct CtkWritePlan {
    int kernel;
    int rb;
    int sub;
    int kb;
    int tab_batched;
    int64_t nchunk;
    unsigned grid;
    size_t lds;
    int64_t shape;
};
inline CtkWritePlan ctk_write_plan(int64_t T, int64_t nt, int ny, int nx, int W, bool aligned16)
{
    CtkWritePlan p = {};
    p.rb = ctk_write_rows(T, ny, nx);
    p.nchunk = (ny + p.rb - 1) / p.rb;
    const int64_t nblk4 = nt * p.nchunk;
    p.tab_batched = nblk4 < 200000 ? 1 : 0;
    const size_t tables = ctk_write_tables_lds(p.rb, W), lds4 = tables + (size_t)CTK_RVCAP * 4;
    if (!((nx % 4 == 0) && aligned16 && (int64_t)ny * nx < 0x7fffffff && nblk4 < (1 << 24) && nt > 0 && lds4 <= 60 * 1024)) {
        p.kernel = nt > 0 ? CTK_WR_GENERIC : CTK_WR_NONE;
        p.grid = (unsigned)ctk_grid_for_rows(nt * ny);
        return p;
    }
    p.grid = (unsigned)nblk4;
    const size_t tab5 = tables + (((size_t)CTK_RV5 * 4 + 15) & ~(size_t)15) + 16;
    auto rows_per_image = [&](int kb) { int q = p.rb; while (q > 1 && tab5 + (size_t)q * nx * 4 > (size_t)kb * 1024) q--; return q; };
    p.kb = 20;
    p.sub = rows_per_image(p.kb);
    if ((p.rb + p.sub - 1) / p.sub > 2)
        for (int kb = 24; kb <= 28; kb += 4) {
            const int s2 = rows_per_image(kb);
            if ((p.rb + s2 - 1) / s2 <= 2) { p.kb = kb; p.sub = s2; break; }
        }
    p.lds = tab5 + (size_t)p.sub * nx * 4;
    if (p.lds <= (size_t)p.kb * 1024) {
        p.kernel = CTK_WR_V5;
        p.shape = ((int64_t)p.rb << 24) | ((int64_t)p.sub << 8) | (p.tab_batched ? 1 : 2) | (4 << (p.kb / 4 - 5));
    } else {
        p.kernel = CTK_WR_V4; p.sub = 0; p.kb = 0;
        p.lds = lds4;
        p.shape = (int64_t)p.rb << 24;
    }
    return p;
}
inline bool ctk_write_chunk_copy(const CtkWritePlan &whole_shard) { return whole_shard.kernel >= CTK_WR_V4 && whole_shard.nchunk <= CTK_CV_MAXCHUNK; }

inline int ctk_runval_threads(CtkPath path, int64_t T, uint64_t total_runs, int forced)
{
    if (path != CTK_PATH_FUSED) return 256;
    if (forced > 0) return forced;
    return (T > 65536 && total_runs / (uint64_t)T < 1024) ? 64 : 256;
}
inline int64_t ctk_runval_code(int threads, bool chunk_copy) { return threads * 10 + (chunk_copy ? 1 : 0); }
inline int ctk_compact_init_threads(CtkPath path, int64_t T, int forced)
{
// ... 565 lines not shown
```

### contrack_amd/csrc/ctk_kernels.hip

```cpp
#include <utility>
#include <hip/hip_runtime.h>
#include <type_traits>
#include <stdint.h>
#include "ctk_tables.h"
#include "ctk_device.h"

#define WAVE 64
#define FULL64 0xffffffffffffffffull

__device__ __forceinline__ int lane_id() { return (int)(threadIdx.x & (WAVE - 1)); }

__device__ __forceinline__ void ctk_zf_set(uint32_t *counters, uint32_t key) { counters[CTK_ZF_OFF + (key & (CTK_ZF_SLOTS - 1)) * CTK_ZF_STRIDE] = 1u; }
__device__ __forceinline__ void ctk_zf_reset(uint32_t *counters, int64_t i) { if (i < CTK_ZF_SLOTS) counters[CTK_ZF_OFF + i * CTK_ZF_STRIDE] = 0u; }
__device__ __forceinline__ uint32_t ctk_zf_mine(const uint32_t *counters, int tid, int nthreads)
{
    uint32_t v = 0;
    for (int i = tid; i < CTK_ZF_SLOTS; i += nthreads) v |= __hip_atomic_load(&counters[CTK_ZF_OFF + i * CTK_ZF_STRIDE], __ATOMIC_RELAXED, __HIP_MEMORY_SCOPE_AGENT);
    return v;
}

__device__ __forceinline__ uint32_t wave_incl_scan_u32(uint32_t v)
{
    int lane = lane_id();
#pragma unroll
    for (int d = 1; d < WAVE; d <<= 1) {
        uint32_t o = __shfl_up(v, d);
        if (lane >= d) v += o;
    }
    return v;
}

__device__ __forceinline__ uint32_t wave_sum_u32(uint32_t v)
{
#pragma unroll
    for (int d = WAVE / 2; d > 0; d >>= 1) v += __shfl_xor(v, d);
    return v;
}

__device__ __forceinline__ uint64_t shfl_up_u64(uint64_t v, int d)
{
    uint32_t lo = __shfl_up((uint32_t)v, d), hi = __shfl_up((uint32_t)(v >> 32), d);
    return ((uint64_t)hi << 32) | lo;
}
__device__ __forceinline__ uint64_t shfl_down_u64(uint64_t v, int d)
{
    uint32_t lo = __shfl_down((uint32_t)v, d), hi = __shfl_down((uint32_t)(v >> 32), d);
    return ((uint64_t)hi << 32) | lo;
}
__device__ __forceinline__ uint64_t shfl_u64(uint64_t v, int src)
{
    uint32_t lo = __shfl((uint32_t)v, src), hi = __shfl((uint32_t)(v >> 32), src);
    return ((uint64_t)hi << 32) | lo;
}

__device__ __forceinline__ uint32_t block_excl_scan(uint32_t v, uint32_t *sm, uint32_t *total)
{
    int lane = lane_id(), wv = (int)(threadIdx.x >> 6), nw = (int)(blockDim.x >> 6);
    uint32_t inc = wave_incl_scan_u32(v);
    __syncthreads();
    if (lane == WAVE - 1) sm[wv] = inc;
    __syncthreads();
    uint32_t base = 0, tot = 0;
    for (int i = 0; i < nw; i++) {
        uint32_t s = sm[i];
        if (i < wv) base += s;
        tot += s;
    }
    *total = tot;
    return base + inc - v;
}

__device__ __forceinline__ uint32_t uf_find(uint32_t *p, uint32_t i)
{
    uint32_t cur = __hip_atomic_load(&p[i], __ATOMIC_RELAXED, __HIP_MEMORY_SCOPE_WORKGROUP);
    if (cur == i) return i;
    uint32_t prev = i;
    for (;;) {
        const uint32_t next = __hip_atomic_load(&p[cur], __ATOMIC_RELAXED, __HIP_MEMORY_SCOPE_WORKGROUP);
        if (next == cur) return cur;
        __hip_atomic_store(&p[prev], next, __ATOMIC_RELAXED, __HIP_MEMORY_SCOPE_WORKGROUP);
        prev = cur;
        cur = next;
    }
}
__device__ __forceinline__ void uf_unite(uint32_t *p, uint32_t a, uint32_t b)
{
    for (;;) {
        a = uf_find(p, a);
// ... 481 lines not shown
    }
    __syncthreads();
    uint64_t base = base_ptr ? (uint64_t)*base_ptr : 0ull;
    if (base_ptr && tid == 0) out[-1] = 0u;
    for (int i = 0; i < wv; i++) base += wsum[i];
    uint64_t run = base + inc - s;
    for (int64_t i = b; i < e; i++) { out[i] = (uint32_t)run; run += in[i]; }
    if (tid == 1023) {
        out[n] = (uint32_t)run;
        if (run > 0xffffffffull) atomicOr(ovf, CTK_OVF_RUNS);
        if (mail) {
            uint32_t m = 0;
            for (int i = 0; i < 16; i++) m = max(m, wmax[i]);
            mail[0] = (uint32_t)run; mail[1] = m; mail[2] = run > 0xffffffffull ? CTK_OVF_RUNS : 0u; mail[3] = n > 0 ? in[n - 1] : 0u;
            if (stamp) { __threadfence_system(); __hip_atomic_store(&mail[4], stamp, __ATOMIC_RELEASE, __HIP_MEMORY_SCOPE_SYSTEM); }
        }
    }
}

#define CTK_SCAN_BLOCK 1024
__global__ __launch_bounds__(CTK_SCAN_BLOCK) void k_scan_blocks_sum(const uint32_t *__restrict__ in, int64_t n, uint64_t *__restrict__ bsum, uint32_t *__restrict__ bmax)
{
    __shared__ uint64_t ws[CTK_SCAN_BLOCK / 64];
    __shared__ uint32_t wm[CTK_SCAN_BLOCK / 64];
    const int64_t i = (int64_t)blockIdx.x * CTK_SCAN_BLOCK + threadIdx.x;
    const uint32_t v = i < n ? in[i] : 0u;
    uint64_t s = v;
    uint32_t m = v;
    for (int o = 32; o > 0; o >>= 1) { s += (uint64_t)__shfl_xor((unsigned long long)s, o); m = max(m, (uint32_t)__shfl_xor((int)m, o)); }
    if (lane_id() == 0) { ws[threadIdx.x >> 6] = s; wm[threadIdx.x >> 6] = m; }
    __syncthreads();
    if (threadIdx.x == 0) {
        uint64_t t = 0; uint32_t mm = 0;
        for (int k = 0; k < CTK_SCAN_BLOCK / 64; k++) { t += ws[k]; mm = max(mm, wm[k]); }
        bsum[blockIdx.x] = t; bmax[blockIdx.x] = mm;
    }
}
__global__ __launch_bounds__(CTK_SCAN_BLOCK) void k_scan_blocks(const uint32_t *__restrict__ in, int64_t n, uint32_t *__restrict__ out, uint32_t *ovf,
                                                                const uint64_t *__restrict__ bsum, const uint32_t *__restrict__ bmax, uint32_t *mail, uint32_t stamp)
{
    __shared__ uint64_t ws[CTK_SCAN_BLOCK / 64];
    __shared__ uint32_t wm[CTK_SCAN_BLOCK / 64];
    __shared__ uint64_t sbase;
    const int tid = (int)threadIdx.x, lane = lane_id(), wv = tid >> 6;
    const int nb = (int)gridDim.x, b = (int)blockIdx.x;
    uint64_t s = 0;
    uint32_t m = 0;
    for (int k = tid; k < b; k += CTK_SCAN_BLOCK) s += bsum[k];
    if (b == nb - 1 && mail) for (int k = tid; k < nb; k += CTK_SCAN_BLOCK) m = max(m, bmax[k]);
    for (int o = 32; o > 0; o >>= 1) { s += (uint64_t)__shfl_xor((unsigned long long)s, o); m = max(m, (uint32_t)__shfl_xor((int)m, o)); }
    if (lane == 0) { ws[wv] = s; wm[wv] = m; }
    __syncthreads();
    if (tid == 0) { uint64_t t = 0; for (int k = 0; k < CTK_SCAN_BLOCK / 64; k++) t += ws[k]; sbase = t; }
    __syncthreads();
    const uint64_t base = sbase;
    uint32_t mall = 0;
    for (int k = 0; k < CTK_SCAN_BLOCK / 64; k++) mall = max(mall, wm[k]);
    __syncthreads();
    const int64_t i = (int64_t)b * CTK_SCAN_BLOCK + tid;
    const uint32_t v = i < n ? in[i] : 0u;
    const uint64_t inc = wave_incl_scan_u64((uint64_t)v);
    if (lane == WAVE - 1) ws[wv] = inc;
    __syncthreads();
    uint64_t run = base + inc - v;
    for (int k = 0; k < wv; k++) run += ws[k];
    if (i < n) out[i] = (uint32_t)run;
    if (b == nb - 1 && i == n - 1) {
        const uint64_t total = run + v;
        out[n] = (uint32_t)total;
        if (total > 0xffffffffull) atomicOr(ovf, CTK_OVF_RUNS);
        if (mail) {
            mail[0] = (uint32_t)total; mail[1] = mall; mail[2] = total > 0xffffffffull ? CTK_OVF_RUNS : 0u; mail[3] = v;
            if (stamp) { __threadfence_system(); __hip_atomic_store(&mail[4], stamp, __ATOMIC_RELEASE, __HIP_MEMORY_SCOPE_SYSTEM); }
        }
    }
}

struct Label2dArgs {
    const uint64_t *mask;
    const uint16_t *wstart;
    const uint32_t *rowstart;
    const uint32_t *run_base;
    uint32_t *run_comp;
    uint32_t *ncomp;
    uint32_t *cs_mrep;
    uint32_t *cs_box;
    int64_t *cs_area;
    CtkSeam *seams;
    uint32_t *seam_cnt;
    uint32_t *counters;
    const int64_t *wlo, *whi;
    int ny, nx, W;
    uint32_t lds_cap;
    uint32_t cap_runs;
    uint16_t *g_x0, *g_x1, *g_y;
    uint32_t *g_parent, *g_root, *g_idmap;
};

#ifdef CTK_PHASE_TIMING
__device__ unsigned long long g_phase_t[16];
#define PHASE_MARK(k) do { __syncthreads(); if (threadIdx.x == 0 && blockIdx.x == gridDim.x / 2) g_phase_t[k] = wall_clock64(); } while (0)
#else
#define PHASE_MARK(k) do { } while (0)
#endif

template <int NW> struct L2dPrefetch { uint16_t w[NW > 0 ? NW : 1]; };

template <int THREADS, typename IT , int LDS_COMPS, int NW = 0>
__device__ __forceinline__ void label2d_body(const Label2dArgs &a, const int t, const uint32_t nruns,
                                             uint16_t *x0, uint16_t *x1, uint16_t *yrow, uint32_t *parent,
                                             IT *root, IT *idmap, IT *rs ,
                                             uint32_t *sm_scan, const uint64_t *mrow ,
                                             const bool mrow_staged ,
                                             void *lds_tab ,
                                             const uint32_t rbase, const L2dPrefetch<NW> &pf)
{
    const int tid = (int)threadIdx.x;
    const int ny = a.ny, nx = a.nx, W = a.W;

    PHASE_MARK(0);
    if (NW == 0) {
        for (int y = tid; y < ny; y += THREADS) rs[y] = (IT)a.rowstart[(int64_t)t * ny + y];
        if (tid == 0) rs[ny] = (IT)nruns;
    }
    __syncthreads();

    PHASE_MARK(1);
    {
        const uint16_t *wglob = a.wstart + (int64_t)t * ny * W;
        const uint64_t *mglob = a.mask + (int64_t)t * ny * W;
        const int nwords = ny * W;
        auto extract = [&](int k, int y, int w, uint64_t m, uint64_t left, uint64_t right, uint32_t wpre) {
            (void)k;
            const uint64_t cin = (w > 0) ? (left >> 63) : 0ull;
            const uint64_t nin = (w + 1 < W) ? (right & 1ull) : 0ull;
            uint64_t starts = m & ~((m << 1) | cin);
            uint64_t ends = m & ~((m >> 1) | (nin << 63));
            const uint32_t nbefore = rs[y] + wpre;
            uint32_t si = nbefore, ei = nbefore - (uint32_t)(cin & m & 1ull);
            const int xb = w * 64;
            while (starts) {
                int b = __builtin_ctzll(starts);
                starts &= starts - 1;
                x0[si] = (uint16_t)(xb + b);
                yrow[si] = (uint16_t)y;
                parent[si] = si;
                si++;
            }
            while (ends) {
                int b = __builtin_ctzll(ends);
                ends &= ends - 1;
                x1[ei] = (uint16_t)(xb + b);
                ei++;
            }
        };
        const int dq = THREADS / W, dr = THREADS - dq * W;
        int yk = tid / W, wk = tid - yk * W;
        if (NW > 0) {
#pragma unroll
            for (int u = 0; u < (NW > 0 ? NW : 1); u++) {
                const int k = tid + u * THREADS;
                if (k >= nwords) break;
                const int y = yk, w = wk;
                yk += dq; wk += dr;
                if (wk >= W) { wk -= W; yk++; }
                const uint64_t m = mrow[k];
// ... 40 lines not shown
        if (y == 0) continue;
        uint32_t lo = rs[y - 1], hi = rs[y];
        if (lo == hi) continue;
        const int xa = (int)x0[r] - 1, xb = (int)x1[r] + 1;
        uint32_t l = lo, h = hi;
        while (l < h) {
            uint32_t m = (l + h) >> 1;
            if ((int)x1[m] < xa) l = m + 1; else h = m;
        }
        for (uint32_t s = l; s < hi && (int)x0[s] <= xb; s++) uf_unite(parent, r, s);
    }
    __syncthreads();

    PHASE_MARK(3);
    uint32_t ncomp = 0;
    {
        const uint32_t per = (nruns + THREADS - 1) / THREADS, rb = min(nruns, (uint32_t)tid * per), re = min(nruns, rb + per);
        uint32_t v = 0, tot;
        for (uint32_t r = rb; r < re; r++) { const uint32_t q = uf_find(parent, r); root[r] = (IT)q; v += (q == r) ? 1u : 0u; }
        uint32_t ex = block_excl_scan(v, sm_scan, &tot);
        for (uint32_t r = rb; r < re; r++) if (root[r] == r) idmap[r] = (IT)(ex++);
        ncomp = tot;
    }
    PHASE_MARK(4);
    if (tid == 0) a.ncomp[t] = ncomp;
    uint32_t *cmrep = a.cs_mrep + rbase;
    uint32_t *gbox = a.cs_box + (int64_t)rbase * 4;
    int64_t *garea = a.cs_area + (int64_t)rbase * 2;
    const bool tab_lds = lds_tab != nullptr && ncomp <= (uint32_t)LDS_COMPS;
    int64_t *carea = tab_lds ? (int64_t *)lds_tab : garea;
    uint32_t *cbox = tab_lds ? (uint32_t *)((int64_t *)lds_tab + 2 * LDS_COMPS) : gbox;
    for (uint32_t c = tid; c < ncomp; c += THREADS) {
        parent[c] = c;
        cbox[c * 4 + 0] = 0xffffu; cbox[c * 4 + 1] = 0u; cbox[c * 4 + 2] = 0xffffu; cbox[c * 4 + 3] = 0u;
        carea[c * 2] = 0; carea[c * 2 + 1] = 0;
    }
    __syncthreads();

    PHASE_MARK(5);
    {
        uint32_t carry = 0;
        CtkSeam *out = a.seams + (int64_t)t * ny;
        for (int y0 = 0; y0 < ny; y0 += THREADS) {
            const int y = y0 + tid;
            uint32_t f = 0, l = 0, v = 0, cf = 0, cl = 0;
            if (y < ny) {
                f = rs[y]; l = rs[y + 1];
                if (f != l) {
                    l--;
                    v = (x0[f] == 0 && x1[l] == (uint16_t)(nx - 1)) ? 1u : 0u;
                    if (v) {
                        cf = idmap[root[f]]; cl = idmap[root[l]];
                        if (cf != cl) uf_unite(parent, cf, cl);
                    }
                }
            }
            uint32_t tot;
            const uint32_t ex = block_excl_scan(v, sm_scan, &tot);
            if (v) {
                CtkSeam q;
                q.t = (uint32_t)t; q.y = (uint32_t)y; q.cl = cf; q.cr = cl;
                out[carry + ex] = q;
            }
            carry += tot;
        }
        if (tid == 0) a.seam_cnt[t] = carry;
    }
    PHASE_MARK(6);
    constexpr int TBN = THREADS == 1024 ? 2 : 4;
    for (uint32_t r0 = tid; r0 < nruns; r0 += TBN * THREADS) {
        int yy[TBN];
        int64_t wl[TBN], wh[TBN];
#pragma unroll
        for (int j = 0; j < TBN; j++) yy[j] = yrow[min(r0 + (uint32_t)j * THREADS, nruns - 1u)];
#pragma unroll
        for (int j = 0; j < TBN; j++) { wl[j] = a.wlo[yy[j]]; wh[j] = a.whi[yy[j]]; }
#pragma unroll
        for (int j = 0; j < TBN; j++) {
            const uint32_t r = r0 + (uint32_t)j * THREADS;
            if (r >= nruns) break;
            const uint32_t rt = root[r];
            const uint32_t c = idmap[rt];
            a.run_comp[rbase + r] = c;
            const int y = yy[j];
            const int64_t len = (int64_t)x1[r] - (int64_t)x0[r] + 1;
            const uint32_t cm = uf_find(parent, c);
            atomicAdd((unsigned long long *)&carea[cm * 2], (unsigned long long)(len * wl[j]));
            atomicAdd((unsigned long long *)&carea[cm * 2 + 1], (unsigned long long)(len * wh[j]));
            atomicMin(&cbox[c * 4 + 0], (uint32_t)y);
            atomicMax(&cbox[c * 4 + 1], (uint32_t)y);
            atomicMin(&cbox[c * 4 + 2], (uint32_t)x0[r]);
            atomicMax(&cbox[c * 4 + 3], (uint32_t)x1[r]);
            if (rt == r) cmrep[c] = cm;
        }
    }
    if (tab_lds) {
        __syncthreads();
        for (uint32_t i = tid; i < ncomp * 4; i += THREADS) gbox[i] = cbox[i];
        for (uint32_t i = tid; i < ncomp * 2; i += THREADS) garea[i] = carea[i];
    }
    PHASE_MARK(7);
    PHASE_MARK(8);
}


template <int RUNS, int COMPS, int RUNS_BELOW, int THREADS, int NYCAP = CTK_LDS_NY>
__global__ __launch_bounds__(THREADS, (THREADS == 1024 || NYCAP < CTK_LDS_NY) ? 8 : 1) void k_label2d_lds(Label2dArgs a)
{
    const int t = (int)blockIdx.x;
#ifdef CTK_PHASE_TIMING
    if (threadIdx.x == 0 && blockIdx.x == gridDim.x / 2) g_phase_t[15] = wall_clock64();
    if (threadIdx.x == 0 && blockIdx.x == 0) g_phase_t[14] = wall_clock64();
    if (threadIdx.x == 0 && blockIdx.x == gridDim.x - 1) g_phase_t[13] = wall_clock64();
#endif
    __shared__ uint16_t x0[RUNS], x1[RUNS], yrow[RUNS], root[RUNS], idmap[RUNS];
    __shared__ uint32_t parent[RUNS];
    __shared__ uint16_t rs[NYCAP + 2];
    __shared__ uint64_t mlds[COMPS * 4];
    __shared__ uint32_t sm_scan[THREADS / 64 + 1];
    const int nwords = a.ny * a.W;
    const uint64_t *mg = a.mask + (int64_t)t * nwords;
    constexpr int NW = (COMPS * 4 + THREADS - 1) / THREADS;
    if (THREADS < 1024 && nwords <= COMPS * 4 && NW <= 8) {
        const uint32_t rb0 = a.run_base[t], rb1 = a.run_base[t + 1];
        const uint16_t *wg = a.wstart + (int64_t)t * nwords;
        const uint32_t *rg = a.rowstart + (int64_t)t * a.ny;
        uint64_t mreg[NW];
        uint32_t rreg[NW];
        L2dPrefetch<NW> pf;
#pragma unroll
        for (int u = 0; u < NW; u++) {
            const int k = min((int)threadIdx.x + u * THREADS, nwords - 1);
            mreg[u] = mg[k];
            pf.w[u] = wg[k];
            rreg[u] = rg[min((int)threadIdx.x + u * THREADS, a.ny - 1)];
        }
        const uint32_t nruns = rb1 - rb0;
        if (nruns > RUNS || (int64_t)nruns <= (int64_t)RUNS_BELOW || a.ny > NYCAP) return;
        if (rb1 > a.cap_runs) return;
        if (nruns == 0) {
            if (threadIdx.x == 0) { a.ncomp[t] = 0; a.seam_cnt[t] = 0; }
            return;
        }
#pragma unroll
        for (int u = 0; u < NW; u++) {
            const int k = (int)threadIdx.x + u * THREADS;
            if (k < nwords) mlds[k] = mreg[u];
            if (k < a.ny) rs[k] = (uint16_t)rreg[u];
        }
        if (threadIdx.x == 0) rs[a.ny] = (uint16_t)nruns;
        label2d_body<THREADS, uint16_t, COMPS, NW>(a, t, nruns, x0, x1, yrow, parent, root, idmap, rs, sm_scan, mlds, true, mlds, rb0, pf);
        return;
    }
    const uint32_t nruns = a.run_base[t + 1] - a.run_base[t];
    if (nruns > RUNS || (int64_t)nruns <= (int64_t)RUNS_BELOW || a.ny > NYCAP) return;
    if (a.run_base[t + 1] > a.cap_runs) return;
    if (nruns == 0) {
        if (threadIdx.x == 0) { a.ncomp[t] = 0; a.seam_cnt[t] = 0; }
        return;
    }
    label2d_body<THREADS, uint16_t, COMPS>(a, t, nruns, x0, x1, yrow, parent, root, idmap, rs, sm_scan, mg, false, mlds, a.run_base[t], L2dPrefetch<0>());
}

__global__ __launch_bounds__(256) void k_label2d_glb(Label2dArgs a, uint32_t *g_rs )
{
    const int t = (int)blockIdx.x;
// ... 85 lines not shown
        ci.F[2 * (int64_t)g] = 0; ci.F[2 * (int64_t)g + 1] = 0;
        ci.B[2 * (int64_t)g] = 0; ci.B[2 * (int64_t)g + 1] = 0;
        ci.keep0[g] = 1; ci.keep1[g] = 1;
        ci.touch[g] = 0;
        ci.parent[g] = g;
        if (ci.ovr_slot) ci.ovr_slot[g] = 0;
    }
    __syncthreads();
    for (uint32_t c = tid; c < n; c += blockDim.x) {
        const uint32_t y0 = cs_box[(int64_t)(rb + c) * 4], y1 = cs_box[(int64_t)(rb + c) * 4 + 1];
        if (ci.next_tiny[y0] <= (int32_t)y1) ci.touch[cb + cs_mrep[rb + c]] = 1u;
    }
    if (t == 0) {
        for (int i = tid; i < ci.nchanged; i += blockDim.x) ci.changed[i] = 0u;
        if (tid == 0) { *ci.ambig = 0u; if (ci.amb_cnt) *ci.amb_cnt = 0u; if (ci.dcount) *ci.dcount = 0u; }
    }
    if (ci.pstate && tid == 0) { ci.pstate[(size_t)t * ci.pstride] = 0u; if (t == ci.T - 1) ci.pstate[(size_t)ci.T * ci.pstride] = 0u; }
}

__global__ __launch_bounds__(256) void k_compact_seams(const CtkSeam *__restrict__ scratch, const uint32_t *__restrict__ seam_cnt,
                                                       const uint32_t *__restrict__ seam_off, int ny, CtkSeam *__restrict__ out)
{
    const int t = (int)blockIdx.x;
    const uint32_t n = seam_cnt[t], o = seam_off[t];
    for (uint32_t i = threadIdx.x; i < n; i += blockDim.x) out[o + i] = scratch[(int64_t)t * ny + i];
}

#define CTK_HASH_SLOTS 512
#define CTK_HASH_PROBES 12

struct OverlapArgs {
    const uint64_t *mask;
    const uint16_t *wstart;
    const uint32_t *rowstart;
    const uint32_t *run_base;
    const uint32_t *run_comp;
    const uint64_t *halo_mask;
    const uint16_t *halo_wstart;
    const uint32_t *halo_rowstart;
    const uint32_t *halo_run_comp;
    int has_prev;
    CtkPair *pairs;
    uint32_t pair_cap;
    uint32_t *pair_base, *pair_cnt;
    uint32_t *counters;
    const int64_t *wlo, *whi;
    int ny, nx, W;
    const uint32_t *cprefix, *mrep;
    uint32_t *p_rc, *p_rd, *p_gc, *p_gd;
    int64_t *F;
    uint32_t pslot;
    uint32_t upair_cap;
};
struct OverlapArgsSeg : OverlapArgs {
    const uint8_t *seg_edge;
};
template <bool SEG, typename A>
__device__ __forceinline__ bool seg_first(const A &a, int t)
{
    if constexpr (SEG) return (a.seg_edge[t] & 1u) != 0;
    else return false;
}

__device__ __forceinline__ void pair_prepare(const OverlapArgs &a, uint32_t slot, uint32_t cb, uint32_t db, uint32_t c, uint32_t d, int64_t lo, int64_t hi)
{
    const uint32_t gc = cb + c, gd = db + d;
    const uint32_t rd = db + a.mrep[gd];
    a.p_gc[slot] = gc; a.p_gd[slot] = gd; a.p_rc[slot] = cb + a.mrep[gc]; a.p_rd[slot] = rd;
    atomicAdd((unsigned long long *)&a.F[2 * (int64_t)rd], (unsigned long long)lo);
    atomicAdd((unsigned long long *)&a.F[2 * (int64_t)rd + 1], (unsigned long long)hi);
}

__device__ __forceinline__ void emit_pair(const OverlapArgs &a, uint32_t t, uint32_t c, uint32_t d, int64_t lo, int64_t hi, uint32_t cb = 0, uint32_t db = 0)
{
    uint32_t i = atomicAdd(&a.counters[CTK_CNT_UPAIRS], 1u);
    if (i < a.upair_cap) {
        CtkPair p;
        p.t = t; p.c = c; p.d = d; p.pad = 0; p.lo = lo; p.hi = hi;
        a.pairs[a.pair_cap - 1u - i] = p;
        if (a.p_rc) pair_prepare(a, a.pair_cap - 1u - i, cb, db, c, d, lo, hi);
    } else atomicOr(&a.counters[CTK_CNT_OVERFLOW], CTK_OVF_PAIRS);
}

template <int OVB, int THREADS = 256, int WPE = 1 , bool SEG = false>
__global__ __launch_bounds__(THREADS, WPE) void k_overlap(std::conditional_t<SEG, OverlapArgsSeg, OverlapArgs> a)
{
    const int t = (int)blockIdx.x;
    if ((t == 0 && !a.has_prev) || (SEG && seg_first<SEG>(a, t))) {
        if (threadIdx.x == 0) { a.pair_base[t] = 0; a.pair_cnt[t] = 0; }
        return;
    }
    const int tid = (int)threadIdx.x;
    const int ny = a.ny, W = a.W;
    const uint32_t cbc = a.p_rc ? a.cprefix[t] : 0u, cbd = a.p_rc ? a.cprefix[t - 1] : 0u;
    __shared__ unsigned long long hkey[CTK_HASH_SLOTS];
    __shared__ long long hlo[CTK_HASH_SLOTS], hhi[CTK_HASH_SLOTS];
    __shared__ uint32_t sm_scan[THREADS / 64 + 1];
    __shared__ uint32_t out_base;
    for (int i = tid; i < CTK_HASH_SLOTS; i += THREADS) { hkey[i] = FULL64; hlo[i] = 0; hhi[i] = 0; }
    __syncthreads();

    const int nwords = ny * W;
    const uint64_t *mc = a.mask + (int64_t)t * nwords;
    const uint16_t *wsc = a.wstart + (int64_t)t * nwords;
    const uint32_t *rsc = a.rowstart + (int64_t)t * ny;
    const uint32_t *rcc = a.run_comp + a.run_base[t];
    const uint64_t *mp;
    const uint16_t *wsp;
    const uint32_t *rsp, *rcp;
    if (t == 0) { mp = a.halo_mask; wsp = a.halo_wstart; rsp = a.halo_rowstart; rcp = a.halo_run_comp; }
    else {
        mp = a.mask + (int64_t)(t - 1) * nwords; wsp = a.wstart + (int64_t)(t - 1) * nwords;
        rsp = a.rowstart + (int64_t)(t - 1) * ny; rcp = a.run_comp + a.run_base[t - 1];
    }
    auto insert = [&](uint32_t cc, uint32_t cd, int64_t lo, int64_t hi) {
        const unsigned long long key = ((unsigned long long)cc << 32) | cd;
        uint32_t h = (uint32_t)((key * 0x9E3779B97F4A7C15ull) >> 40) & (CTK_HASH_SLOTS - 1);
        for (int q = 0; q < CTK_HASH_PROBES; q++) {
            const unsigned long long old = atomicCAS(&hkey[h], FULL64, key);
            if (old == FULL64 || old == key) {
                atomicAdd((unsigned long long *)&hlo[h], (unsigned long long)lo);
                atomicAdd((unsigned long long *)&hhi[h], (unsigned long long)hi);
                return;
            }
            h = (h + 1) & (CTK_HASH_SLOTS - 1);
        }
        emit_pair(a, (uint32_t)t, cc, cd, lo, hi, cbc, cbd);
    };
    const int lane = tid & 63;
    const int dq = THREADS / W, dr = THREADS - dq * W;
    int yk = tid / W, wk = tid - yk * W;
    for (int i0 = tid; i0 < nwords; i0 += THREADS * OVB) {
        uint64_t c[OVB], p[OVB];
        uint32_t ec[OVB], ep[OVB], lt[OVB];
        uint32_t ltc[OVB], ltp[OVB];
        int yy[OVB];
        uint32_t first = 0;
#pragma unroll
        for (int u = 0; u < OVB; u++) {
            const int idx = i0 + u * THREADS, ii = min(idx, nwords - 1), im = max(ii - 1, 0);
            const int y = min(yk, ny - 1);
            if (wk == 0) first |= 1u << u;
            yk += dq; wk += dr;
            if (wk >= W) { wk -= W; yk++; }
            yy[u] = idx < nwords ? y : -1;
            c[u] = mc[ii]; p[u] = mp[ii];
            const int il = lane == 0 ? 2 * im + 1 : 1;
            ltc[u] = reinterpret_cast<const uint32_t *>(mc)[il];
            ltp[u] = reinterpret_cast<const uint32_t *>(mp)[il];
            ec[u] = rsc[y] + wsc[ii]; ep[u] = rsp[y] + wsp[ii];
        }
#pragma unroll
        for (int u = 0; u < OVB; u++) {
            const uint32_t mine = (uint32_t)(c[u] >> 63) | ((uint32_t)(p[u] >> 63) << 1);
            const uint32_t left = (uint32_t)__shfl_up((int)mine, 1);
            lt[u] = lane != 0 ? left : ((ltc[u] >> 31) | ((ltp[u] >> 31) << 1));
            if ((first >> u) & 1u) lt[u] = 0;
            if (yy[u] < 0) c[u] = 0ull;
        }
        uint32_t cc0[OVB], cd0[OVB];
        int64_t wl[OVB], wh[OVB];
        auto starts = [&](int u, uint64_t &sc, uint64_t &sp) {
            sc = c[u] & ~((c[u] << 1) | (uint64_t)(lt[u] & 1u)); sp = p[u] & ~((p[u] << 1) | (uint64_t)(lt[u] >> 1));
        };
#pragma unroll
        for (int u = 0; u < OVB; u++) {
            const uint64_t o = c[u] & p[u];
            cc0[u] = 0; cd0[u] = 0; wl[u] = 0; wh[u] = 0;
            if (o == 0ull) continue;
            uint64_t sc, sp;
            starts(u, sc, sp);
            const int b = __builtin_ctzll(o);
            const uint64_t below = (b + 1 >= 64) ? FULL64 : ((1ull << (b + 1)) - 1ull);
            cc0[u] = rcc[ec[u] + (uint32_t)__popcll(sc & below) - 1u];
            cd0[u] = rcp[ep[u] + (uint32_t)__popcll(sp & below) - 1u];
            wl[u] = a.wlo[yy[u]]; wh[u] = a.whi[yy[u]];
        }
#pragma unroll
        for (int u = 0; u < OVB; u++) {
            uint64_t ou = c[u] & p[u];
            if (ou == 0ull) continue;
            int b = __builtin_ctzll(ou);
            uint64_t sh = ou >> b;
            int n = (~sh == 0ull) ? 64 : __builtin_ctzll(~sh);
            insert(cc0[u], cd0[u], (int64_t)n * wl[u], (int64_t)n * wh[u]);
            ou = (n >= 64 - b) ? 0ull : (ou & ~(((1ull << n) - 1ull) << b));
            if (ou == 0ull) continue;
            uint64_t sc, sp;
            starts(u, sc, sp);
            while (ou) {
                b = __builtin_ctzll(ou);
                sh = ou >> b;
                n = (~sh == 0ull) ? 64 : __builtin_ctzll(~sh);
                const uint64_t below = (b + 1 >= 64) ? FULL64 : ((1ull << (b + 1)) - 1ull);
                const uint32_t cc = rcc[ec[u] + (uint32_t)__popcll(sc & below) - 1u], cd = rcp[ep[u] + (uint32_t)__popcll(sp & below) - 1u];
                insert(cc, cd, (int64_t)n * wl[u], (int64_t)n * wh[u]);
                ou = (n >= 64 - b) ? 0ull : (ou & ~(((1ull << n) - 1ull) << b));
            }
        }
    }
    __syncthreads();
    {
        uint32_t mine = 0;
        for (int i = tid; i < CTK_HASH_SLOTS; i += THREADS) mine += (hkey[i] != FULL64) ? 1u : 0u;
        uint32_t tot;
        const uint32_t ex = block_excl_scan(mine, sm_scan, &tot);
        if (tid == 0) {
            if (a.pslot) {
                out_base = (uint32_t)t * a.pslot;
                a.pair_base[t] = out_base;
                a.pair_cnt[t] = min(tot, a.pslot);
            } else {
                out_base = tot ? atomicAdd(&a.counters[CTK_CNT_PAIRS], tot) : 0u;
                a.pair_base[t] = out_base;
                a.pair_cnt[t] = (tot && out_base + tot <= a.pair_cap) ? tot : 0u;
                if (tot && out_base + tot > a.pair_cap) atomicOr(&a.counters[CTK_CNT_OVERFLOW], CTK_OVF_PAIRS);
            }
        }
        __syncthreads();
        uint32_t j = out_base + ex;
        const uint32_t jend = a.pslot ? out_base + a.pslot : a.pair_cap;
        for (int i = tid; i < CTK_HASH_SLOTS; i += THREADS) {
            if (hkey[i] == FULL64) continue;
            if (a.pslot && j >= jend) {
                emit_pair(a, (uint32_t)t, (uint32_t)(hkey[i] >> 32), (uint32_t)hkey[i], hlo[i], hhi[i], cbc, cbd);
                j++;
                continue;
            }
            if (j < jend) {
                CtkPair p;
                p.t = (uint32_t)t; p.c = (uint32_t)(hkey[i] >> 32); p.d = (uint32_t)hkey[i]; p.pad = 0;
                p.lo = hlo[i]; p.hi = hhi[i];
                a.pairs[j] = p;
                if (a.p_rc) pair_prepare(a, j, cbc, cbd, p.c, p.d, p.lo, p.hi);
            }
            j++;
        }
    }
}

struct FoldArgs {
    const CtkOp *ops;
    const int32_t *first;
    const int32_t *next;
    int32_t nops;
};

__device__ inline int32_t fold_pixel(const FoldArgs &f, int32_t l, int32_t t, int32_t y, int32_t x)
{
    int32_t s = 0;
    for (;;) {
        bool moved = false;
        for (int32_t idx = f.first[l]; idx >= 0; idx = f.next[idx]) {
            if (idx < s) continue;
            const CtkOp o = f.ops[idx];
            if (t >= o.t0 && t <= o.t1 && y >= o.y0 && y <= o.y1 && x >= o.x0 && x <= o.x1) {
                l = o.lo; s = idx + 1; moved = true; break;
            }
        }
        if (!moved) return l;
    }
}

template <typename F>
__device__ __forceinline__ void for_each_fg_pixel_in_row(const uint64_t *mw, int W, uint32_t rowstart, F f)
{
    const int lane = lane_id();
    uint32_t base = rowstart;
    uint64_t carry = 0;
    for (int w0 = 0; w0 < W; w0 += WAVE) {
        const int wn = min(WAVE, W - w0);
        uint64_t m = (lane < wn) ? mw[w0 + lane] : 0ull;
        uint64_t pm = shfl_up_u64(m, 1);
        uint64_t st = m & ~((m << 1) | ((lane == 0) ? carry : (pm >> 63)));
        uint32_t n = (uint32_t)__popcll(st);
        uint32_t inc = wave_incl_scan_u32(n);
        uint32_t before = base + inc - n;
        for (int k = 0; k < wn; k++) {
            uint64_t mk = shfl_u64(m, k);
            if (mk == 0ull) continue;
            uint64_t sk = shfl_u64(st, k);
            uint32_t bk = __shfl(before, k);
            if ((mk >> lane) & 1ull) {
                uint64_t below = (lane == 63) ? FULL64 : ((1ull << (lane + 1)) - 1ull);
                f((w0 + k) * 64 + lane, bk + (uint32_t)__popcll(sk & below) - 1u);
            }
        }
        base += __shfl(inc, WAVE - 1);
        carry = shfl_u64(m, wn - 1) >> 63;
    }
}

__device__ inline int32_t comp_final_label(const FoldArgs &f, int32_t l, int32_t t, int q0, int q1, int q2, int q3 )
{
    if (f.nops == 0) return l;
    int32_t cur = l, s = 0;
    for (;;) {
        bool again = false;
        for (int32_t idx = f.first[cur]; idx >= 0; idx = f.next[idx]) {
            if (idx < s) continue;
            const CtkOp o = f.ops[idx];
            const bool t_in = t >= o.t0 && t <= o.t1;
            const bool inside = t_in && q0 >= o.y0 && q1 <= o.y1 && q2 >= o.x0 && q3 <= o.x1;
            const bool disjoint = !t_in || q1 < o.y0 || q0 > o.y1 || q3 < o.x0 || q2 > o.x1;
            if (inside) { cur = o.lo; s = idx + 1; again = true; break; }
            if (!disjoint) return -l;
        }
        if (!again) return cur;
    }
}

__device__ __forceinline__ bool ctk_guard_bad(const uint32_t *guard)
{
    return guard && ((guard[CTK_CNT_OVERFLOW] & CTK_OVF_PAIRS) != 0u || guard[CTK_CNT_POISON] != 0u);
}

struct ExtentArgs {
    const uint32_t *guard;
    const uint64_t *mask;
    const uint32_t *rowstart;
    const uint32_t *run_base;
// ... 832 lines not shown
```

### include/contrack_hip.h

```cpp
#ifndef CONTRACK_HIP_H
#define CONTRACK_HIP_H

#include <stddef.h>
#include <stdint.h>

#ifdef __cplusplus
extern "C" {
#endif

#define CTK_OK            0
#define CTK_E_INVALID    -1
#define CTK_E_NODEVICE   -2
#define CTK_E_NOMEM      -3
#define CTK_E_RANGE      -4
#define CTK_E_INTERNAL   -5
#define CTK_E_STATE      -6
#define CTK_E_COMM       -7

typedef struct ctk_handle ctk_handle;

int         ctk_version(void);
const char *ctk_last_error(void);
int         ctk_device_count(void);
int         ctk_create(ctk_handle **h, int device);
// ... 76 lines not shown
int  ctk_track_sharded_seg_f32_dev(ctk_handle *h, ctk_comm *c, const float *anom_dev, int64_t T_local, int64_t t_begin, int64_t T_total,
                                   int ny, int nx, const double *thr , int cmp_op, const float *wrow, double overlap,
                                   int persistence, int twosided, int32_t *flag_dev, int64_t *n_tracked, const int64_t *starts_global,
                                   int64_t nseg);
int  ctk_track_sharded_seg_f64_dev(ctk_handle *h, ctk_comm *c, const double *anom_dev, int64_t T_local, int64_t t_begin, int64_t T_total,
                                   int ny, int nx, const double *thr, int cmp_op, const float *wrow, double overlap,
                                   int persistence, int twosided, int32_t *flag_dev, int64_t *n_tracked, const int64_t *starts_global,
                                   int64_t nseg);

typedef int (*ctk_read_chunk_fn)(void *user, int64_t t0, int64_t nt, void *dst);
typedef int (*ctk_write_chunk_fn)(void *user, int64_t t0, int64_t nt, const int32_t *src);
int ctk_track_stream_f32(ctk_handle *h, const float *anom, int64_t T, int ny, int nx, const double *thr, int cmp_op, const float *wrow,
                         double overlap, int persistence, int twosided, int32_t *flag, int64_t *n_tracked, int64_t chunk_steps);
int ctk_track_stream_f64(ctk_handle *h, const double *anom, int64_t T, int ny, int nx, const double *thr, int cmp_op, const float *wrow,
                         double overlap, int persistence, int twosided, int32_t *flag, int64_t *n_tracked, int64_t chunk_steps);
int ctk_track_stream_cb(ctk_handle *h, int elem_bytes , int64_t T, int ny, int nx, ctk_read_chunk_fn reader,
                        void *reader_user, const double *thr, int cmp_op, const float *wrow, double overlap, int persistence, int twosided,
                        ctk_write_chunk_fn writer, void *writer_user, int64_t *n_tracked, int64_t chunk_steps);
int ctk_track_stream_seg_f32(ctk_handle *h, const float *anom, int64_t T, int ny, int nx, const double *thr, int cmp_op, const float *wrow,
                             double overlap, int persistence, int twosided, int32_t *flag, int64_t *n_tracked, int64_t chunk_steps,
                             const int64_t *starts, int64_t nseg);
int ctk_track_stream_seg_f64(ctk_handle *h, const double *anom, int64_t T, int ny, int nx, const double *thr, int cmp_op, const float *wrow,
                             double overlap, int persistence, int twosided, int32_t *flag, int64_t *n_tracked, int64_t chunk_steps,
                             const int64_t *starts, int64_t nseg);
int ctk_track_stream_seg_cb(ctk_handle *h, int elem_bytes , int64_t T, int ny, int nx, ctk_read_chunk_fn reader,
                            void *reader_user, const double *thr, int cmp_op, const float *wrow, double overlap, int persistence,
                            int twosided, ctk_write_chunk_fn writer, void *writer_user, int64_t *n_tracked, int64_t chunk_steps,
                            const int64_t *starts, int64_t nseg);
int ctk_stream_times(ctk_handle *h, double *ms4);

#define CTK_K_THRESHOLD 0
#define CTK_K_SCAN      1
#define CTK_K_LABEL2D   2
#define CTK_K_OVERLAP   3
#define CTK_K_EXTENT    4
#define CTK_K_RUNLABEL  5
#define CTK_K_RELABEL   6
#define CTK_K_RESOLVE   7
#define CTK_K_RESOLVE2  8
#define CTK_K_COUNT     9
#define CTK_T_HOST_RESOLVE 10
#define CTK_T_D2H          11
#define CTK_T_H2D          12
#define CTK_T_TOTAL        13
#define CTK_NTIMERS        14
int ctk_set_timing(ctk_handle *h, int level);
int ctk_get_timing_sums(ctk_handle *h, double *sums, int64_t *counts, int reset);
#define CTK_S_RUNS          0
#define CTK_S_MAX_RUNS_STEP 1
#define CTK_S_COMPONENTS    2
#define CTK_S_PAIRS         3
#define CTK_S_SEAM_ROWS     4
#define CTK_S_LABELS        5
#define CTK_S_OPS           6
#define CTK_S_FILTER_PASSES 7
#define CTK_S_HOST_PATH     8
#define CTK_S_UPAIRS        12
#define CTK_S_PAIR_REGROW   13
#define CTK_S_FILTER_ROUNDS 14
#define CTK_S_EXACT_FIXUPS  16
#define CTK_S_AMBIGUOUS     15
#define CTK_S_HOST_REASON   18
#define CTK_S_SHARED_ROWS   17
#define CTK_S_RELABEL_KERNEL 19
#define CTK_S_FUSED         20
#define CTK_S_X4_SPECULATED 21
#define CTK_S_RLE_OUT       22
#define CTK_S_MASK_TRIES    23
#define CTK_S_MASK_RATIO    24
#define CTK_NSTATS          25
int ctk_get_stats(ctk_handle *h, int64_t *out );
#define CTK_S_MASK_CHECK_US 25
#define CTK_S_MASK_SPACER_MB 26
#define CTK_S_LABEL_FORMS   27
#define CTK_S_OVERLAP_FORM  28
#define CTK_S_ROWCOUNT_THREADS 29
#define CTK_S_FILTER_FORMS  30
#define CTK_S_EXTENT_FORM   31
#define CTK_S_RUNVAL_FORM   32
#define CTK_S_RELABEL_SHAPE 33
#define CTK_S_COUNT_FORM    34
#define CTK_S_DEVICE_CUS    35
#define CTK_S_ROWCOUNT_GROUPS 36
#define CTK_NSTATS_ALL      40
int ctk_get_stats_n(ctk_handle *h, int64_t *out, int n);
int ctk_get_timings(ctk_handle *h, double *ms );

int ctk_dev_malloc(ctk_handle *h, void **p, size_t nbytes);
int ctk_dev_free(ctk_handle *h, void *p);
int ctk_memcpy_h2d(ctk_handle *h, void *dst_dev, const void *src, size_t nbytes);
int ctk_memcpy_d2h(ctk_handle *h, void *dst, const void *src_dev, size_t nbytes);
int ctk_sync(ctk_handle *h);
int ctk_host_alloc(ctk_handle *h, void **p, size_t nbytes);
int ctk_host_free(ctk_handle *h, void *p);
int ctk_set_result_transfer(ctk_handle *h, int mode);
int ctk_host_register(ctk_handle *h, void *p, size_t nbytes);
int ctk_host_unregister(ctk_handle *h, void *p);
void *ctk_stream(ctk_handle *h);
int ctk_dev_memset(ctk_handle *h, void *p_dev, int byte, size_t nbytes);

typedef struct ctk_life_row {
    int32_t t, label, shift, pad;
    double area, swv, swvy, swvx;
} ctk_life_row;
int ctk_lifecycle_f32_dev(ctk_handle *h, const int32_t *flag_dev, const float *field_dev, int64_t T, int ny, int nx, const float *wrow, int64_t *nrows);
int ctk_lifecycle_f64_dev(ctk_handle *h, const int32_t *flag_dev, const double *field_dev, int64_t T, int ny, int nx, const float *wrow, int64_t *nrows);
int ctk_lifecycle_f32(ctk_handle *h, const int32_t *flag, const float *field, int64_t T, int ny, int nx, const float *wrow, int64_t *nrows);
int ctk_lifecycle_f64(ctk_handle *h, const int32_t *flag, const double *field, int64_t T, int ny, int nx, const float *wrow, int64_t *nrows);
int ctk_lifecycle_rows(ctk_handle *h, ctk_life_row *rows, int64_t cap);
typedef struct ctk_life_exact {
    double area, swv, s, sy, sx;
} ctk_life_exact;
int ctk_lifecycle_exact(ctk_handle *h, const int64_t *row_idx, int64_t n, ctk_life_exact *out);
typedef int (*ctk_life_pick_fn)(void *user, const ctk_life_row *rows, int64_t n, int64_t *idx, int64_t *nidx);
int ctk_lifecycle_stream_f32(ctk_handle *h, const int32_t *flag, const float *field, int64_t T, int ny, int nx, const float *wrow, int64_t chunk_steps,
                             ctk_life_pick_fn pick, void *pick_user, int64_t *nrows, int64_t *nexact);
int ctk_lifecycle_stream_f64(ctk_handle *h, const int32_t *flag, const double *field, int64_t T, int ny, int nx, const float *wrow, int64_t chunk_steps,
                             ctk_life_pick_fn pick, void *pick_user, int64_t *nrows, int64_t *nexact);
int ctk_lifecycle_stream_cb(ctk_handle *h, int elem_bytes , int64_t T, int ny, int nx, ctk_read_chunk_fn flag_reader,
                            void *flag_user, ctk_read_chunk_fn field_reader, void *field_user, const float *wrow, int64_t chunk_steps,
                            ctk_life_pick_fn pick, void *pick_user, int64_t *nrows, int64_t *nexact);
int ctk_lifecycle_stream_exact(ctk_handle *h, int64_t *row_idx, ctk_life_exact *out, int64_t cap);

int ctk_anom_f32(ctk_handle *h, const float *x, int64_t T, int ny, int nx, const int32_t *group, int ngroups, int window, int smooth,
                 const float *clim_in, float *anom_out, float *clim_out, int keep_resident);
int ctk_anom_f64(ctk_handle *h, const double *x, int64_t T, int ny, int nx, const int32_t *group, int ngroups, int window, int smooth,
                 const double *clim_in, double *anom_out, double *clim_out, int keep_resident);
int ctk_anom_seg_f32(ctk_handle *h, const float *x, int64_t T, int ny, int nx, const int32_t *group, int ngroups, int window, int smooth,
                     const float *clim_in, float *anom_out, float *clim_out, int keep_resident, const int64_t *starts, int64_t nseg);
int ctk_anom_seg_f64(ctk_handle *h, const double *x, int64_t T, int ny, int nx, const int32_t *group, int ngroups, int window, int smooth,
                     const double *clim_in, double *anom_out, double *clim_out, int keep_resident, const int64_t *starts, int64_t nseg);
typedef int (*ctk_write_values_fn)(void *user, int64_t t0, int64_t nt, const void *src);
int ctk_anom_stream_f32(ctk_handle *h, const float *x, int64_t T, int ny, int nx, const int32_t *group, int ngroups, int window, int smooth,
                        const int64_t *starts, int64_t nseg, const float *clim_in, float *anom_out, float *clim_out, int64_t chunk_steps);
int ctk_anom_stream_f64(ctk_handle *h, const double *x, int64_t T, int ny, int nx, const int32_t *group, int ngroups, int window, int smooth,
                        const int64_t *starts, int64_t nseg, const double *clim_in, double *anom_out, double *clim_out, int64_t chunk_steps);
int ctk_anom_stream_cb(ctk_handle *h, int elem_bytes , int64_t T, int ny, int nx, ctk_read_chunk_fn reader, void *reader_user,
                       const int32_t *group, int ngroups, int window, int smooth, const int64_t *starts, int64_t nseg, const void *clim_in,
                       void *clim_out, ctk_write_values_fn writer, void *writer_user, int64_t chunk_steps);
int ctk_resident_anom(ctk_handle *h, int64_t *T, int *ny, int *nx, int *is_f64);
int ctk_resident_anom_generation(ctk_handle *h, uint64_t *generation);
int ctk_track_resident(ctk_handle *h, const double *thr, int cmp_op, const float *wrow, double overlap, int persistence, int twosided,
                       int32_t *flag, int64_t *n_tracked);
int ctk_percentile_f32(ctk_handle *h, const float *x, int64_t T, int ny, int nx, int y0, int y1, double q, double *out);
int ctk_percentile_f64(ctk_handle *h, const double *x, int64_t T, int ny, int nx, int y0, int y1, double q, double *out);
int ctk_percentile_groups_f32(ctk_handle *h, const float *x, int64_t T, int ny, int nx, int y0, int y1, const int32_t *group, int ngroups, int window,
                              double q, double *out );
int ctk_percentile_groups_f64(ctk_handle *h, const double *x, int64_t T, int ny, int nx, int y0, int y1, const int32_t *group, int ngroups, int window,
                              double q, double *out );
int ctk_percentile_field_f32(ctk_handle *h, const float *x, int64_t T, int ny, int nx, int y0, int y1, const int32_t *group, int ngroups, int window,
                             double q, double *out );
int ctk_percentile_field_f64(ctk_handle *h, const double *x, int64_t T, int ny, int nx, int y0, int y1, const int32_t *group, int ngroups, int window,
                             double q, double *out );
int ctk_std_field_f32(ctk_handle *h, const float *x, int64_t T, int ny, int nx, int y0, int y1, const int32_t *group, int ngroups, int window,
                      int ddof, int skipna, double *out_std , double *out_mean ,
                      uint32_t *out_n );
int ctk_std_field_f64(ctk_handle *h, const double *x, int64_t T, int ny, int nx, int y0, int y1, const int32_t *group, int ngroups, int window,
                      int ddof, int skipna, double *out_std , double *out_mean ,
                      uint32_t *out_n );

int ctk_level_mean_f32(ctk_handle *h, const float *x, int64_t steps, int nlev, int ny, int nx, const double *weights, int skipna, float *out, int keep_resident);
int ctk_level_mean_f64(ctk_handle *h, const double *x, int64_t steps, int nlev, int ny, int nx, const double *weights, int skipna, double *out, int keep_resident);
int ctk_level_mean_f32_dev(ctk_handle *h, const float *x_dev, int64_t steps, int nlev, int ny, int nx, const double *weights, int skipna, float *out_dev);
int ctk_level_mean_f64_dev(ctk_handle *h, const double *x_dev, int64_t steps, int nlev, int ny, int nx, const double *weights, int skipna, double *out_dev);
int ctk_level_mean_stream_f32(ctk_handle *h, const float *x, int64_t steps, int nlev, int ny, int nx, const double *weights, int skipna, float *out,
                              int64_t chunk_steps, int keep_resident);
// ... 156 lines not shown
```

### include/contrack_hip_debug.h

```cpp
#ifndef CONTRACK_HIP_DEBUG_H
#define CONTRACK_HIP_DEBUG_H

#include "contrack_hip.h"

#ifdef __cplusplus
extern "C" {
#endif

int  ctk_debug_fail_at(ctk_handle *h, int stage);

int ctk_debug_mask(ctk_handle *h, uint8_t *mask );

int ctk_debug_label2d(ctk_handle *h, int before_seam, int32_t *lab );

int ctk_debug_set_pair_capacity(ctk_handle *h, uint32_t records);

double ctk_debug_np_sum(const double *a, size_t n);

int ctk_debug_boundary_resolve(int world, const int32_t *nlast, const int32_t *nh, const int32_t *nroots, const int32_t *last_flat,
                               const int32_t *halo_flat, int64_t *off , int32_t *last_label_flat, int32_t *halo_label_flat,
                               int32_t *n_absorbed );
int ctk_debug_boundary_resolve_breaks(int world, const int32_t *nlast, const int32_t *nh, const int32_t *nroots, const int32_t *last_flat,
                                      const int32_t *halo_flat, int64_t *off , int32_t *last_label_flat,
                                      int32_t *halo_label_flat, int32_t *n_absorbed , int32_t *n_crossing);

int ctk_debug_set_seam_caps(ctk_handle *h, int labels, int ops);

int ctk_debug_shard_exchange(ctk_handle *h, int64_t *out12);

int ctk_debug_set_shared_ops_reserve(ctk_handle *h, int64_t n);

int ctk_debug_set_mailbox(ctk_handle *h, uint32_t cand_records, uint32_t labels);

int ctk_debug_set_spin(ctk_handle *h, double limit_ms, int stall_mode);

int ctk_debug_stream_ceiling(ctk_handle *h, void *p_dev, size_t nbytes, int mode, int reps, double *best_ms);

int ctk_debug_time_relabel(ctk_handle *h, int32_t *flag_dev, int persistence, int variant, int xcd, int reps, double *ms);

int ctk_debug_set_small_threads(ctk_handle *h, int extent, int run_values, int compact_init);

typedef struct ctk_form_query { int64_t T, nt, ny, nx, f64, aligned16, field, max_runs_step, total_runs, n_labels, last_nlab, async_passes, no_sys, n_cus, seg, pslot, path, forced_extent, forced_run_values, forced_compact_init, spec_set, launched; } ctk_form_query;
typedef struct ctk_form_plan { int64_t thr_kind, thr_u7, thr_rbt, thr_grid, rowcount_threads, v0b, v0_ok, v0_runs, need_glb, spec_launched, spec_bits, missing, missing_bits, next_spec, overlap_form, extent_form, write_kernel, write_rb, write_sub, write_kb, write_batched, write_lds, write_grid, write_shape, chunk_copy, runval_threads, compact_init_threads, count_staged, count_fused, filter_sys, filter_passes, filter_blk, filter_two_pc, filter_nb, filter_unite, filter_merged, filter_bits, filter_bits_sync, round_blk, round_two_pc, round_nb, rowcount_groups; } ctk_form_plan;
int ctk_debug_forms(const ctk_form_query *q, ctk_form_plan *p);

int ctk_debug_live(int64_t *out4);

int ctk_debug_io_bytes(ctk_handle *h, int64_t *out4);

int ctk_set_filter_round(ctk_handle *h, int passes);

int ctk_set_fused_pass(ctk_handle *h, int enable);

int ctk_set_device_resolve(ctk_handle *h, int enable);

int ctk_synth_fill(ctk_handle *h, float *anom_dev, int64_t T, int ny, int nx, uint64_t seed);

int ctk_synth_fill_window(ctk_handle *h, float *anom_dev, int64_t t0, int64_t T, int ny, int nx, uint64_t seed);

int ctk_checksum_i32_dev(ctk_handle *h, const int32_t *p_dev, int64_t n, int64_t index0, uint64_t *out2);

int ctk_check_flag_dev(ctk_handle *h, const float *anom_dev, const int32_t *flag_dev, int64_t T, int ny, int nx, const double *thr, int cmp_op,
                       int persistence, int64_t max_id, uint64_t *out6);

int ctk_expand_runs_host(const uint64_t *mask, const uint32_t *rowstart, const uint32_t *run_base, const int32_t *run_val, int64_t T, int ny, int nx,
                         int32_t *flag, int *wrote_background, int *complex_runs);

int ctk_debug_set_freq(ctk_handle *h, int64_t slice, int nt);
int ctk_debug_time_freq(ctk_handle *h, const int32_t *flag_dev, int64_t T, int ny, int nx, const int32_t *group, int ngroups, int32_t above,
                        uint32_t *counts_dev, int reps, double *ms2);

int ctk_debug_set_spell(ctk_handle *h, int64_t slice);
int ctk_debug_time_spell(ctk_handle *h, const int32_t *flag_dev, int64_t T, int ny, int nx, const int32_t *group, int ngroups, const int64_t *seg_starts,
                         int64_t nseg, int32_t above, int by_id, int64_t min_duration, uint32_t *events_dev, uint32_t *steps_dev, uint32_t *longest_dev,
                         int reps, double *ms2);

int ctk_debug_percentile_values(ctk_handle *h, double *out, int64_t n);

int ctk_debug_percentile_groups_sweeps(ctk_handle *h, int64_t *sweeps);
int ctk_debug_percentile_groups_plan(int keybits, int64_t nband, int ngroups, int window, int64_t max_steps_of_a_group, int64_t *out22);
int ctk_debug_percentile_groups_state(ctk_handle *h, int ngroups, uint32_t *nu_day, uint32_t *need, uint64_t *n_of);
int ctk_debug_time_percentile_groups(ctk_handle *h, const float *x_dev, int64_t T, int ny, int nx, int y0, int y1, const int32_t *group, int ngroups,
                                     int window, double q, int reps, double *out, double *ms12);

int ctk_debug_anom_form(ctk_handle *h, int64_t *form);
int ctk_debug_anom_plan(int elem_bytes, int smooth, int64_t nt, int64_t npix, int64_t waves_wanted, int64_t grid_y_max, int64_t *out5);
int ctk_debug_set_anom(ctk_handle *h, int64_t waves_wanted, int64_t grid_y_max);
int ctk_debug_anom_launch(ctk_handle *h, int64_t *out8);

int ctk_debug_filter_plan(int elem_bytes, int K, int64_t stride, int64_t nout, int64_t npix, int64_t waves_wanted, int64_t grid_y_max, int forced, int64_t *out6);
int ctk_debug_set_filter(ctk_handle *h, int64_t waves_wanted, int64_t grid_y_max, int forced);
int ctk_debug_filter_launch(ctk_handle *h, int64_t *out9);
int ctk_debug_time_filter(ctk_handle *h, const void *x_dev, int is_f64, int64_t T, int ny, int nx, const double *w, int K, int64_t stride, int64_t offset,
                          int edges, int skipna, void *out_dev, int64_t T_out, int64_t copy_bytes, int reps, double *ms2);

int ctk_debug_percentile_field_plan(int keybytes, int64_t max_pool_steps, int ngroups, int window, int64_t *out4);
int ctk_debug_percentile_field_form(ctk_handle *h, int64_t *out2);
int ctk_debug_time_percentile_field(ctk_handle *h, const void *x_dev, int is_f64, int64_t T, int ny, int nx, int y0, int y1, const int32_t *group,
                                    int ngroups, int window, double q, int reps, double *out, double *out_direct, double *ms4);

int ctk_debug_std_field_plan(int ngroups, int window, int skipna, int64_t *out4);
int ctk_debug_std_field_form(ctk_handle *h, int64_t *out2);
int ctk_debug_time_std_field(ctk_handle *h, const void *x_dev, int is_f64, int64_t T, int ny, int nx, int y0, int y1, const int32_t *group,
                             int ngroups, int window, int ddof, int skipna, int reps, double *out_std, double *ms2);

int ctk_debug_lifecycle_plan(int64_t T, int ny, int nx, int f64, int64_t flag_align, int64_t field_align, int64_t *out5);
int ctk_debug_lifecycle_path(ctk_handle *h, int64_t *out8, uint8_t *steps, int64_t T);

int ctk_debug_level_plan(int elem_bytes, int64_t nsel, int64_t npix, int64_t steps, int aligned, int64_t *out7);
int ctk_debug_set_level(ctk_handle *h, int xcd_mode, int64_t grid_max);
int ctk_debug_level_form(ctk_handle *h, int64_t *out2);
int ctk_debug_time_level_mean(ctk_handle *h, const void *x_dev, int is_f64, int64_t steps, int nlev, int ny, int nx, const double *weights, int skipna,
                              void *out_dev, int reps, double *ms2);

int ctk_debug_reversal_plan(int elem_bytes, int64_t ny, int64_t nx, int64_t steps, int aligned, int64_t *out6);
int ctk_debug_set_reversal(ctk_handle *h, int xcd_mode, int64_t grid_max);
int ctk_debug_reversal_form(ctk_handle *h, int64_t *out2);
int ctk_debug_time_reversal(ctk_handle *h, const void *x_dev, int is_f64, int64_t steps, int ny, int nx, const int32_t *eq, const int32_t *po, const int32_t *eq2,
                            const double *dE, const double *tS, const double *tN, const double *tS2, int mask, void *out_dev, int reps, double *ms2);

int ctk_debug_subset_plan(int by_row, int64_t max_id, int64_t longest, int want_hits, int64_t ny, int64_t nx, int64_t steps, int aligned, int64_t grid_max,
                          int64_t *out12);
int ctk_debug_set_subset(ctk_handle *h, int xcd_mode, int64_t grid_max);
// ... 41 lines not shown
```

Baseline: 5.947 million.

## Compute temporal overlap by merging per-row run records instead of bitmask words

During labelling, label2d now writes a compact per-run record (packed x0/x1 and component id) alongside run_comp. A new k_overlap_rows kernel computes the overlap between consecutive timesteps with a batched two-pointer merge over each row's run lists, replacing the scan over mask words. It feeds the existing LDS hash table and the flush, which are factored out into shared helpers. It is used only when there is no previous chunk, T<=1024 and ny*W>=8192. It costs an extra record buffer and extra global writes in label2d, and each thread walks a whole row serially.

```diff
diff --git a/contrack_amd/_native.py b/contrack_amd/_native.py
--- a/contrack_amd/_native.py
+++ b/contrack_amd/_native.py
@@ -256,6 +256,23 @@
     p = FormPlan()
     check(lib().ctk_debug_forms(C.byref(q), C.byref(p)))
     return {n: getattr(p, n) for n, _ in FormPlan._fields_}
+
+
+def row_overlap(rec_c, rec_p):
+    c = np.ascontiguousarray(rec_c, dtype=np.uint32).reshape(-1, 2)
+    p = np.ascontiguousarray(rec_p, dtype=np.uint32).reshape(-1, 2)
+    cap = len(c) + len(p) + 1
+    out = np.zeros((cap, 3), dtype=np.uint32)
+    n = C.c_int64(0)
+    check(lib().ctk_debug_row_overlap(c.ctypes.data, len(c), p.ctypes.data, len(p), out.ctypes.data, cap, C.byref(n)))
+    assert n.value <= cap
+    return out[:n.value]
+
+
+def overlap_rows_plan(T, ny, nx, has_prev=False, records_valid=True):
+    v = np.zeros(4, dtype=np.int64)
+    check(lib().ctk_debug_overlap_rows_plan(int(T), int(ny), int(nx), int(bool(has_prev)), int(bool(records_valid)), v.ctypes.data))
+    return dict(rows=int(v[0]), can=int(v[1]), batch=int(v[2]), threads=int(v[3]))
 
 
 def debug_live():
@@ -2021,14 +2038,17 @@
         return v is None or (mt is not None and int(mt.group(0)) != 0)
 
     def stats(self):
-        v = np.zeros(37, dtype=np.int64)
-        check(lib().ctk_get_stats_n(self._h, v.ctypes.data, 37))
+        v = np.zeros(38, dtype=np.int64)
+        check(lib().ctk_get_stats_n(self._h, v.ctypes.data, 38))
         names = ["runs", "max_runs_per_step", "components", "pairs", "seam_rows_to_driver", "labels_3d", "seam_ops",
                  "filter_passes", "host_path", "seam_loop_ns", "seam_folds", "seam_copy_ns", "ungrouped_pairs", "pair_table_regrows", "filter_rounds",
                  "ambiguous_decisions", "exact_fixups", "shared_seam_rows", "off_fused_path_reason", "relabel_kernel", "fused_pass", "x4_speculated", "result_as_runs", "mask_allocations_tried", "mask_ratio_x1000",
                  "mask_check_us", "mask_spacer_mb", "label_forms", "overlap_form", "rowcount_threads",
-                 "filter_forms", "extent_form", "runval_form", "relabel_shape", "count_form", "device_cus", "rowcount_groups"]
+                 "filter_forms", "extent_form", "runval_form", "relabel_shape", "count_form", "device_cus", "rowcount_groups", "overlap_rows"]
         return dict(zip(names, v.tolist()))
+
+    def debug_set_overlap_rows(self, mode):
+        check(lib().ctk_debug_set_overlap_rows(self._h, int(mode)))
 
     def debug_set_pair_capacity(self, records):
         check(lib().ctk_debug_set_pair_capacity(self._h, int(records)))
diff --git a/contrack_amd/csrc/ctk_api.hip b/contrack_amd/csrc/ctk_api.hip
--- a/contrack_amd/csrc/ctk_api.hip
+++ b/contrack_amd/csrc/ctk_api.hip
@@ -247,6 +247,7 @@
     uint32_t pair_cap = 0, seam_cap = 0;
     bool need_glb = false;
     DevBuf mask, wstart, rowstart, tcount, run_base, ncomp, cprefix, thr32, wlo, whi, counters;
+    DevBuf run_rec;
     DevBuf run_comp, run_val, cs_mrep, cs_box, cs_area, d_mrep, d_box, d_area, comp_label;
     DevBuf g_x0, g_x1, g_y, g_parent, g_root, g_idmap, g_rs;
     DevBuf pairs, seams, ext, ops, op_first, op_next, op_stage, halo_in, halo_out, dbg;
@@ -388,6 +389,8 @@
     uint64_t spin_limit = CTK_SPIN_LIMIT_TICKS;
     int debug_stall = 0;
     bool no_sys = false, sh_retrying = false;
+    int overlap_rows_mode = 0;
+    bool rec_valid = false;
     int small_threads[3] = {0, 0, 0};
     bool thr_nostore = false;
     bool thr_probe = false;
@@ -640,6 +643,41 @@
     if (extent != 0 && extent != 64 && extent != 128 && extent != 256 && extent != 1024) return ctk_set_error(CTK_E_INVALID, "ctk_debug_set_small_threads: extent 0 / 64 / 128 / 256, or 1024 = k_extent_blk");
     if (!h) return ctk_set_error(CTK_E_INVALID, "null handle");
     h->small_threads[0] = extent; h->small_threads[1] = run_values; h->small_threads[2] = compact_init;
+    return CTK_OK;
+}
+
+extern "C" int ctk_debug_set_overlap_rows(ctk_handle *h, int mode)
+{
+    if (!h || mode < 0 || mode > 2) return ctk_set_error(CTK_E_INVALID, "ctk_debug_set_overlap_rows: null handle, or mode not 0 (the rule), 1 (word form) or 2 (run-level form)");
+    h->overlap_rows_mode = mode;
+    return CTK_OK;
+}
+
+extern "C" int ctk_debug_row_overlap(const uint32_t *rec_c, int64_t nc, const uint32_t *rec_p, int64_t np, uint32_t *out, int64_t cap, int64_t *n_out)
+{
+    if (nc < 0 || np < 0 || cap < 0 || nc > 65536 || np > 65536 || (nc && !rec_c) || (np && !rec_p) || (cap && !out) || !n_out)
+        return ctk_set_error(CTK_E_INVALID, "ctk_debug_row_overlap: null argument, or a list of more than 65 536 runs");
+    static_assert(sizeof(CtkRunRec) == 8 && alignof(CtkRunRec) == 8, "a run record is two uint32");
+    std::vector<CtkRunRec> c((size_t)nc), p((size_t)np);
+    for (int64_t i = 0; i < nc; i++) c[(size_t)i] = CtkRunRec{rec_c[2 * i], rec_c[2 * i + 1]};
+    for (int64_t i = 0; i < np; i++) p[(size_t)i] = CtkRunRec{rec_p[2 * i], rec_p[2 * i + 1]};
+    int64_t n = 0;
+    ctk_row_overlap(c.data(), (uint32_t)nc, p.data(), (uint32_t)np, [&](uint32_t cc, uint32_t cd, uint32_t len) {
+        if (n < cap) { out[3 * n] = cc; out[3 * n + 1] = cd; out[3 * n + 2] = len; }
+        n++;
+    });
+    *n_out = n;
+    return CTK_OK;
+}
+
+extern "C" int ctk_debug_overlap_rows_plan(int64_t T, int ny, int nx, int has_prev, int records_valid, int64_t *out4)
+{
+    if (!out4 || T < 0 || ny < 1 || nx < 1 || ny > 65535 || nx > 65535) return ctk_set_error(CTK_E_INVALID, "ctk_debug_overlap_rows_plan: bad argument");
+    const int W = (nx + 63) / 64;
+    out4[0] = ctk_overlap_rows(T, ny, W, has_prev, records_valid != 0) ? 1 : 0;
+    out4[1] = ctk_overlap_rows_can(has_prev, records_valid != 0) ? 1 : 0;
+    out4[2] = CTK_OVR_BATCH;
+    out4[3] = CTK_OVR_THREADS;
     return CTK_OK;
 }
 
@@ -1071,7 +1109,7 @@
     h->pass_no++;
     h->state = ST_IDLE;
     h->halo_valid = false; h->halo_v2 = c.defer_compact;
-    h->T = T; h->ny = ny; h->nx = nx; h->W = (nx + 63) / 64; h->has_prev = has_prev ? 1 : 0; h->cmp_op = c.cmp_op;
+    h->T = T; h->ny = ny; h->nx = nx; h->W = (nx + 63) / 64; h->has_prev = has_prev ? 1 : 0; h->cmp_op = c.cmp_op; h->rec_valid = false;
     c.W = h->W;
     c.nrows = T * ny;
     c.shape = ctk_label_shape(T, ny, c.W);
@@ -1328,6 +1366,17 @@
     return CTK_OK;
 }
 
+static bool label2d_wants_records(const ctk_handle *h, const Label2dCall &c)
+{
+    if (c.defer_compact) return false;
+    if (h->overlap_rows_mode == 2) return ctk_overlap_rows_can(h->has_prev, true);
+    return h->overlap_rows_mode == 0 && ctk_overlap_rows(c.T, c.ny, c.W, h->has_prev, true);
+}
+static CtkRunRec *label2d_records(const ctk_handle *h, const Label2dCall &c, uint32_t cap_runs)
+{
+    return (label2d_wants_records(h, c) && h->run_rec.p && h->run_rec.cap / sizeof(CtkRunRec) >= cap_runs) ? P<CtkRunRec>(h->run_rec) : nullptr;
+}
+
 static int launch_label2d(ctk_handle *h, Label2dCall &c, const CtkVariantSet &vs, uint32_t cap_runs)
 {
     const int T = (int)c.T;
@@ -1335,6 +1384,8 @@
     Label2dArgs a;
     a.mask = P<uint64_t>(h->mask); a.wstart = P<uint16_t>(h->wstart); a.rowstart = P<uint32_t>(h->rowstart);
     a.run_base = P<uint32_t>(h->run_base); a.run_comp = P<uint32_t>(h->run_comp); a.ncomp = P<uint32_t>(h->ncomp);
+    a.run_rec = label2d_records(h, c, cap_runs);
+    h->rec_valid = a.run_rec != nullptr;
     a.cs_mrep = P<uint32_t>(h->cs_mrep); a.cs_box = P<uint32_t>(h->cs_box); a.cs_area = P<int64_t>(h->cs_area);
     a.seams = P<CtkSeam>(h->seams); a.seam_cnt = P<uint32_t>(h->seam_cnt); a.counters = P<uint32_t>(h->counters);
     a.wlo = P<int64_t>(h->wlo); a.whi = P<int64_t>(h->wlo) + h->ny;
@@ -1437,6 +1488,12 @@
         h->runs_cap = (uint32_t)std::min<size_t>(Rc, 0xffffffffu);
         c.launched = {false, false, false, false, false, false};
         if (c.spec) c.label_forms |= CTK_LABEL_DISCARDED;
+    }
+    if (label2d_wants_records(h, c) && h->run_rec.cap < (size_t)h->runs_cap * sizeof(CtkRunRec)) {
+        if (h->run_rec.p && h->active_comm) CTKCHK(ctk_comm_wait(h->active_comm));
+        h->run_rec.release();
+        if (h->run_rec.alloc((size_t)h->runs_cap * sizeof(CtkRunRec)) != hipSuccess) (void)hipGetLastError();
+        else c.launched = {false, false, false, false, false, false};
     }
     if (c.defer_compact) {
         const size_t Rd = (size_t)h->runs_cap + (size_t)c.ny * ((size_t)c.nx / 2 + 1);
@@ -1635,6 +1692,19 @@
     static_cast<OverlapArgs &>(as) = a;
     as.seg_edge = h->seg_cur;
     const int form = ctk_overlap_form(h->T, h->ny, h->W);
+    h->stats[CTK_S_OVERLAP_FORM] = (as.seg_edge ? CTK_OVERLAP_SEG : 0) + form;
+    const bool rows_can = ctk_overlap_rows_can(h->has_prev, h->rec_valid);
+    const bool rows = h->overlap_rows_mode == 2 ? rows_can : (h->overlap_rows_mode == 0 && ctk_overlap_rows(h->T, h->ny, h->W, h->has_prev, h->rec_valid));
+    h->stats[CTK_S_OVERLAP_ROWS] = rows ? 1 : 0;
+    if (rows) {
+        OverlapRowsArgs ar;
+        static_cast<OverlapArgsSeg &>(ar) = as;
+        ar.run_rec = P<CtkRunRec>(h->run_rec);
+        if (as.seg_edge) k_overlap_rows<CTK_OVR_THREADS, true><<<(int)h->T, CTK_OVR_THREADS, 0, h->stream>>>(ar);
+        else k_overlap_rows<CTK_OVR_THREADS><<<(int)h->T, CTK_OVR_THREADS, 0, h->stream>>>(ar);
+        HIPCHK(hipGetLastError());
+        return CTK_OK;
+    }
 #define CTK_OVERLAP(OVB, TH, WPE)                                                                        \
     case CTK_OVERLAP_CODE(OVB, TH, WPE):                                                                 \
         if (as.seg_edge) k_overlap<OVB, TH, WPE, true><<<(int)h->T, TH, 0, h->stream>>>(as);             \
@@ -1650,7 +1720,6 @@
     default: return ctk_set_error(CTK_E_INTERNAL, "k_overlap: no instance of form %d", form);
     }
 #undef CTK_OVERLAP
-    h->stats[CTK_S_OVERLAP_FORM] = (as.seg_edge ? CTK_OVERLAP_SEG : 0) + form;
     HIPCHK(hipGetLastError());
     return CTK_OK;
 }
diff --git a/contrack_amd/csrc/ctk_device.h b/contrack_amd/csrc/ctk_device.h
--- a/contrack_amd/csrc/ctk_device.h
+++ b/contrack_amd/csrc/ctk_device.h
@@ -31,6 +31,7 @@
 #define CTK_JACOBI_ROUND 10
 #define PB_G 16
 #define CTK_RL_BLOCKS 8192
+#define CTK_OVR_BATCH 4
 
 #define CTK_OVF_PAIRS 1u
 #define CTK_OVF_SEAMS 2u
diff --git a/contrack_amd/csrc/ctk_forms.h b/contrack_amd/csrc/ctk_forms.h
--- a/contrack_amd/csrc/ctk_forms.h
+++ b/contrack_amd/csrc/ctk_forms.h
@@ -125,6 +125,14 @@
     if (per == 5) return CTK_OVERLAP_CODE(5, 256, 1);
     if (per == 6) return CTK_OVERLAP_CODE(6, 256, 1);
     return CTK_OVERLAP_CODE(8, 256, 1);
+}
+
+#define CTK_OVR_THREADS 256
+inline bool ctk_overlap_rows_can(int has_prev, bool records_valid) { return !has_prev && records_valid; }
+inline bool ctk_overlap_rows(int64_t T, int ny, int W, int has_prev, bool records_valid)
+{
+    if (!ctk_overlap_rows_can(has_prev, records_valid)) return false;
+    return T <= 1024 && ny * W >= 8192;
 }
 
 #define CTK_EXTENT_BLK 1024
diff --git a/contrack_amd/csrc/ctk_kernels.hip b/contrack_amd/csrc/ctk_kernels.hip
--- a/contrack_amd/csrc/ctk_kernels.hip
+++ b/contrack_amd/csrc/ctk_kernels.hip
@@ -4,6 +4,7 @@
 #include <stdint.h>
 #include "ctk_tables.h"
 #include "ctk_device.h"
+#include "ctk_rowmerge.h"
 
 #define WAVE 64
 #define FULL64 0xffffffffffffffffull
@@ -651,6 +652,7 @@
     const uint32_t *rowstart;
     const uint32_t *run_base;
     uint32_t *run_comp;
+    CtkRunRec *run_rec;
     uint32_t *ncomp;
     uint32_t *cs_mrep;
     uint32_t *cs_box;
@@ -857,6 +859,7 @@
             const uint32_t rt = root[r];
             const uint32_t c = idmap[rt];
             a.run_comp[rbase + r] = c;
+            if (a.run_rec) a.run_rec[rbase + r] = CtkRunRec{(uint32_t)x0[r] | ((uint32_t)x1[r] << 16), c};
             const int y = yy[j];
             const int64_t len = (int64_t)x1[r] - (int64_t)x0[r] + 1;
             const uint32_t cm = uf_find(parent, c);
@@ -1108,6 +1111,67 @@
     } else atomicOr(&a.counters[CTK_CNT_OVERFLOW], CTK_OVF_PAIRS);
 }
 
+__device__ __forceinline__ void overlap_insert(const OverlapArgs &a, unsigned long long *hkey, long long *hlo, long long *hhi, int t, uint32_t cc,
+                                               uint32_t cd, int64_t lo, int64_t hi, uint32_t cbc, uint32_t cbd)
+{
+    const unsigned long long key = ((unsigned long long)cc << 32) | cd;
+    uint32_t h = (uint32_t)((key * 0x9E3779B97F4A7C15ull) >> 40) & (CTK_HASH_SLOTS - 1);
+    for (int q = 0; q < CTK_HASH_PROBES; q++) {
+        const unsigned long long old = atomicCAS(&hkey[h], FULL64, key);
+        if (old == FULL64 || old == key) {
+            atomicAdd((unsigned long long *)&hlo[h], (unsigned long long)lo);
+            atomicAdd((unsigned long long *)&hhi[h], (unsigned long long)hi);
+            return;
+        }
+        h = (h + 1) & (CTK_HASH_SLOTS - 1);
+    }
+    emit_pair(a, (uint32_t)t, cc, cd, lo, hi, cbc, cbd);
+}
+
+template <int THREADS>
+__device__ __forceinline__ void overlap_flush(const OverlapArgs &a, int t, int tid, const unsigned long long *hkey, const long long *hlo, const long long *hhi,
+                                              uint32_t *sm_scan, uint32_t *out_base_lds, uint32_t cbc, uint32_t cbd)
+{
+    uint32_t mine = 0;
+    for (int i = tid; i < CTK_HASH_SLOTS; i += THREADS) mine += (hkey[i] != FULL64) ? 1u : 0u;
+    uint32_t tot;
+    const uint32_t ex = block_excl_scan(mine, sm_scan, &tot);
+    if (tid == 0) {
+        uint32_t out_base;
+        if (a.pslot) {
+            out_base = (uint32_t)t * a.pslot;
+            a.pair_base[t] = out_base;
+            a.pair_cnt[t] = min(tot, a.pslot);
+        } else {
+            out_base = tot ? atomicAdd(&a.counters[CTK_CNT_PAIRS], tot) : 0u;
+            a.pair_base[t] = out_base;
+            a.pair_cnt[t] = (tot && out_base + tot <= a.pair_cap) ? tot : 0u;
+            if (tot && out_base + tot > a.pair_cap) atomicOr(&a.counters[CTK_CNT_OVERFLOW], CTK_OVF_PAIRS);
+        }
+        *out_base_lds = out_base;
+    }
+    __syncthreads();
+    const uint32_t out_base = *out_base_lds;
+    uint32_t j = out_base + ex;
+    const uint32_t jend = a.pslot ? out_base + a.pslot : a.pair_cap;
+    for (int i = tid; i < CTK_HASH_SLOTS; i += THREADS) {
+        if (hkey[i] == FULL64) continue;
+        if (a.pslot && j >= jend) {
+            emit_pair(a, (uint32_t)t, (uint32_t)(hkey[i] >> 32), (uint32_t)hkey[i], hlo[i], hhi[i], cbc, cbd);
+            j++;
+            continue;
+        }
+        if (j < jend) {
+            CtkPair p;
+            p.t = (uint32_t)t; p.c = (uint32_t)(hkey[i] >> 32); p.d = (uint32_t)hkey[i]; p.pad = 0;
+            p.lo = hlo[i]; p.hi = hhi[i];
+            a.pairs[j] = p;
+            if (a.p_rc) pair_prepare(a, j, cbc, cbd, p.c, p.d, p.lo, p.hi);
+        }
+        j++;
+    }
+}
+
 template <int OVB, int THREADS = 256, int WPE = 1 , bool SEG = false>
 __global__ __launch_bounds__(THREADS, WPE) void k_overlap(std::conditional_t<SEG, OverlapArgsSeg, OverlapArgs> a)
 {
@@ -1139,20 +1203,7 @@
         mp = a.mask + (int64_t)(t - 1) * nwords; wsp = a.wstart + (int64_t)(t - 1) * nwords;
         rsp = a.rowstart + (int64_t)(t - 1) * ny; rcp = a.run_comp + a.run_base[t - 1];
     }
-    auto insert = [&](uint32_t cc, uint32_t cd, int64_t lo, int64_t hi) {
-        const unsigned long long key = ((unsigned long long)cc << 32) | cd;
-        uint32_t h = (uint32_t)((key * 0x9E3779B97F4A7C15ull) >> 40) & (CTK_HASH_SLOTS - 1);
-        for (int q = 0; q < CTK_HASH_PROBES; q++) {
-            const unsigned long long old = atomicCAS(&hkey[h], FULL64, key);
-            if (old == FULL64 || old == key) {
-                atomicAdd((unsigned long long *)&hlo[h], (unsigned long long)lo);
-                atomicAdd((unsigned long long *)&hhi[h], (unsigned long long)hi);
-                return;
-            }
-            h = (h + 1) & (CTK_HASH_SLOTS - 1);
-        }
-        emit_pair(a, (uint32_t)t, cc, cd, lo, hi, cbc, cbd);
-    };
+    auto insert = [&](uint32_t cc, uint32_t cd, int64_t lo, int64_t hi) { overlap_insert(a, hkey, hlo, hhi, t, cc, cd, lo, hi, cbc, cbd); };
     const int lane = tid & 63;
     const int dq = THREADS / W, dr = THREADS - dq * W;
     int yk = tid / W, wk = tid - yk * W;
@@ -1226,43 +1277,46 @@
         }
     }
     __syncthreads();
-    {
-        uint32_t mine = 0;
-        for (int i = tid; i < CTK_HASH_SLOTS; i += THREADS) mine += (hkey[i] != FULL64) ? 1u : 0u;
-        uint32_t tot;
-        const uint32_t ex = block_excl_scan(mine, sm_scan, &tot);
-        if (tid == 0) {
-            if (a.pslot) {
-                out_base = (uint32_t)t * a.pslot;
-                a.pair_base[t] = out_base;
-                a.pair_cnt[t] = min(tot, a.pslot);
-            } else {
-                out_base = tot ? atomicAdd(&a.counters[CTK_CNT_PAIRS], tot) : 0u;
-                a.pair_base[t] = out_base;
-                a.pair_cnt[t] = (tot && out_base + tot <= a.pair_cap) ? tot : 0u;
-                if (tot && out_base + tot > a.pair_cap) atomicOr(&a.counters[CTK_CNT_OVERFLOW], CTK_OVF_PAIRS);
-            }
-        }
-        __syncthreads();
-        uint32_t j = out_base + ex;
-        const uint32_t jend = a.pslot ? out_base + a.pslot : a.pair_cap;
-        for (int i = tid; i < CTK_HASH_SLOTS; i += THREADS) {
-            if (hkey[i] == FULL64) continue;
-            if (a.pslot && j >= jend) {
-                emit_pair(a, (uint32_t)t, (uint32_t)(hkey[i] >> 32), (uint32_t)hkey[i], hlo[i], hhi[i], cbc, cbd);
-                j++;
-                continue;
-            }
-            if (j < jend) {
-                CtkPair p;
-                p.t = (uint32_t)t; p.c = (uint32_t)(hkey[i] >> 32); p.d = (uint32_t)hkey[i]; p.pad = 0;
-                p.lo = hlo[i]; p.hi = hhi[i];
-                a.pairs[j] = p;
-                if (a.p_rc) pair_prepare(a, j, cbc, cbd, p.c, p.d, p.lo, p.hi);
-            }
-            j++;
-        }
-    }
+    overlap_flush<THREADS>(a, t, tid, hkey, hlo, hhi, sm_scan, &out_base, cbc, cbd);
+}
+
+struct OverlapRowsArgs : OverlapArgsSeg {
+    const CtkRunRec *run_rec;
+};
+template <int THREADS, bool SEG = false>
+__global__ __launch_bounds__(THREADS) CTK_SGPR_8WAVES void k_overlap_rows(OverlapRowsArgs a)
+{
+    const int t = (int)blockIdx.x;
+    if (t == 0 || (SEG && seg_first<SEG>(a, t))) {
+        if (threadIdx.x == 0) { a.pair_base[t] = 0; a.pair_cnt[t] = 0; }
+        return;
+    }
+    const int tid = (int)threadIdx.x;
+    const int ny = a.ny;
+    const uint32_t cbc = a.p_rc ? a.cprefix[t] : 0u, cbd = a.p_rc ? a.cprefix[t - 1] : 0u;
+    __shared__ unsigned long long hkey[CTK_HASH_SLOTS];
+    __shared__ long long hlo[CTK_HASH_SLOTS], hhi[CTK_HASH_SLOTS];
+    __shared__ uint32_t sm_scan[THREADS / 64 + 1];
+    __shared__ uint32_t out_base;
+    const uint32_t *rsc = a.rowstart + (int64_t)t * ny, *rsp = a.rowstart + (int64_t)(t - 1) * ny;
+    const uint32_t rb_p = a.run_base[t - 1], rb_c = a.run_base[t], rb_n = a.run_base[t + 1];
+    int y = tid;
+    uint32_t c0 = rsc[min(y, ny - 1)], c1 = rsc[min(y + 1, ny - 1)], p0 = rsp[min(y, ny - 1)], p1 = rsp[min(y + 1, ny - 1)];
+    int64_t wl = a.wlo[min(y, ny - 1)], wh = a.whi[min(y, ny - 1)];
+    for (int i = tid; i < CTK_HASH_SLOTS; i += THREADS) { hkey[i] = FULL64; hlo[i] = 0; hhi[i] = 0; }
+    __syncthreads();
+    while (y < ny) {
+        if (y + 1 >= ny) { c1 = rb_n - rb_c; p1 = rb_c - rb_p; }
+        ctk_row_overlap(a.run_rec + rb_c + c0, c1 - c0, a.run_rec + rb_p + p0, p1 - p0, [&](uint32_t cc, uint32_t cd, uint32_t len) {
+            overlap_insert(a, hkey, hlo, hhi, t, cc, cd, (int64_t)len * wl, (int64_t)len * wh, cbc, cbd);
+        });
+        y += THREADS;
+        if (y >= ny) break;
+        c0 = rsc[y]; c1 = rsc[min(y + 1, ny - 1)]; p0 = rsp[y]; p1 = rsp[min(y + 1, ny - 1)];
+        wl = a.wlo[y]; wh = a.whi[y];
+    }
+    __syncthreads();
+    overlap_flush<THREADS>(a, t, tid, hkey, hlo, hhi, sm_scan, &out_base, cbc, cbd);
 }
 
 struct FoldArgs {
diff --git a/contrack_amd/csrc/ctk_rowmerge.h b/contrack_amd/csrc/ctk_rowmerge.h
--- /dev/null
+++ b/contrack_amd/csrc/ctk_rowmerge.h
@@ -0,0 +1,69 @@
+#pragma once
+#include <stdint.h>
+#include "ctk_device.h"
+
+#if defined(__HIPCC__)
+#define CTK_HD __host__ __device__
+#else
+#define CTK_HD
+#endif
+
+struct alignas(8) CtkRunRec {
+    uint32_t x;
+    uint32_t comp;
+};
+
+struct CtkRowStep {
+    uint32_t len;
+    bool adv_c, adv_p;
+};
+CTK_HD inline CtkRowStep ctk_row_merge_step(uint32_t xc, uint32_t xp)
+{
+    const uint32_t c0 = xc & 0xffffu, c1 = xc >> 16, p0 = xp & 0xffffu, p1 = xp >> 16;
+    const uint32_t lo = c0 > p0 ? c0 : p0, hi = c1 < p1 ? c1 : p1;
+    CtkRowStep s;
+    s.len = hi >= lo ? hi - lo + 1u : 0u;
+    s.adv_c = c1 <= p1;
+    s.adv_p = p1 <= c1;
+    return s;
+}
+
+template <typename Emit>
+CTK_HD inline void ctk_row_overlap(const CtkRunRec *rc, uint32_t nc, const CtkRunRec *rp, uint32_t np, Emit emit)
+{
+    if (nc == 0u || np == 0u) return;
+    constexpr uint32_t B = CTK_OVR_BATCH;
+    CtkRunRec c[B], p[B];
+#pragma unroll
+    for (uint32_t u = 0; u < B; u++) c[u] = rc[u < nc ? u : nc - 1u];
+#pragma unroll
+    for (uint32_t u = 0; u < B; u++) p[u] = rp[u < np ? u : np - 1u];
+    uint32_t ic = nc < B ? nc : B, ip = np < B ? np : B;
+    uint32_t hc = ic, hp = ip;
+    for (;;) {
+        const CtkRowStep s = ctk_row_merge_step(c[0].x, p[0].x);
+        if (s.len) emit(c[0].comp, p[0].comp, s.len);
+        if (s.adv_c) {
+#pragma unroll
+            for (uint32_t u = 0; u + 1 < B; u++) c[u] = c[u + 1];
+            if (--hc == 0u) {
+                if (ic >= nc) break;
+#pragma unroll
+                for (uint32_t u = 0; u < B; u++) c[u] = rc[ic + u < nc ? ic + u : nc - 1u];
+                hc = nc - ic < B ? nc - ic : B;
+                ic += hc;
+            }
+        }
+        if (s.adv_p) {
+#pragma unroll
+            for (uint32_t u = 0; u + 1 < B; u++) p[u] = p[u + 1];
+            if (--hp == 0u) {
+                if (ip >= np) break;
+#pragma unroll
+                for (uint32_t u = 0; u < B; u++) p[u] = rp[ip + u < np ? ip + u : np - 1u];
+                hp = np - ip < B ? np - ip : B;
+                ip += hp;
+            }
+        }
+    }
+}
diff --git a/include/contrack_hip.h b/include/contrack_hip.h
--- a/include/contrack_hip.h
+++ b/include/contrack_hip.h
@@ -182,6 +182,7 @@
 #define CTK_S_COUNT_FORM    34
 #define CTK_S_DEVICE_CUS    35
 #define CTK_S_ROWCOUNT_GROUPS 36
+#define CTK_S_OVERLAP_ROWS  37
 #define CTK_NSTATS_ALL      40
 int ctk_get_stats_n(ctk_handle *h, int64_t *out, int n);
 int ctk_get_timings(ctk_handle *h, double *ms );
diff --git a/include/contrack_hip_debug.h b/include/contrack_hip_debug.h
--- a/include/contrack_hip_debug.h
+++ b/include/contrack_hip_debug.h
@@ -39,6 +39,10 @@
 int ctk_debug_time_relabel(ctk_handle *h, int32_t *flag_dev, int persistence, int variant, int xcd, int reps, double *ms);
 
 int ctk_debug_set_small_threads(ctk_handle *h, int extent, int run_values, int compact_init);
+
+int ctk_debug_set_overlap_rows(ctk_handle *h, int mode);
+int ctk_debug_row_overlap(const uint32_t *rec_c, int64_t nc, const uint32_t *rec_p, int64_t np, uint32_t *out, int64_t cap, int64_t *n_out);
+int ctk_debug_overlap_rows_plan(int64_t T, int ny, int nx, int has_prev, int records_valid, int64_t *out4);
 
 typedef struct ctk_form_query { int64_t T, nt, ny, nx, f64, aligned16, field, max_runs_step, total_runs, n_labels, last_nlab, async_passes, no_sys, n_cus, seg, pslot, path, forced_extent, forced_run_values, forced_compact_init, spec_set, launched; } ctk_form_query;
 typedef struct ctk_form_plan { int64_t thr_kind, thr_u7, thr_rbt, thr_grid, rowcount_threads, v0b, v0_ok, v0_runs, need_glb, spec_launched, spec_bits, missing, missing_bits, next_spec, overlap_form, extent_form, write_kernel, write_rb, write_sub, write_kb, write_batched, write_lds, write_grid, write_shape, chunk_copy, runval_threads, compact_init_threads, count_staged, count_fused, filter_sys, filter_passes, filter_blk, filter_two_pc, filter_nb, filter_unite, filter_merged, filter_bits, filter_bits_sync, round_blk, round_two_pc, round_nb, rowcount_groups; } ctk_form_plan;
```

Result: slower. 5.668 million (-4.7%).
